# hvasbath/beat

Hardware: AMD Instinct MI355X
Metric: SMC chain-steps/s (FFI seismic gfstacking 400 patches x 64 targets x 4096 samples) (higher is better)
Workload: dtype f64; 1 GPU; BASELINE configs[2]: FFI seismic gfstacking, 400 patches x 64 targets x 4096 samples, library (64,400,3,25,4096) f64 = 62.9 GB in HBM, nearest_neighbor, covariance scalar; population SURVEY 8(d): nucleation U over the 20x20 fault, time 0; chains_per_gpu=512, global_chains=512, parallelism=chains sharded over 1 GPU(s), library replicated

## Files before the change

beat_amd/_lib.py:

```python
import ctypes as C
import os

import numpy as np

_HERE = os.path.dirname(os.path.abspath(__file__))
LIB_PATH = os.environ.get("BEATAMD_LIB") or os.path.join(_HERE, "libbeat_amd.so")

NEAREST_NEIGHBOR, MULTILINEAR = 0, 1
W_SCALAR, W_DENSE = 0, 1
STF_HALF_SINUSOID = 0
POL_MTQT, POL_MT, POL_DC = 0, 1, 2
INTERPOLATIONS = {"nearest_neighbor": NEAREST_NEIGHBOR, "multilinear": MULTILINEAR}

OK, EINVAL, EHIP, EINDEX, ENOMEM, ENAN, ENOTPSD, EBADCOV, EOUTSIDE = 0, -1, -2, -3, -4, -5, -6, -7, -8
ABI_VERSION = 120


class BeatAmdError(RuntimeError):
    pass


class FfiLayout(C.Structure):
    _fields_ = [
        ("nparams", C.c_int64),
# ... 6 lines not shown
        ("time_off", C.c_int64),
        ("h_laplacian_off", C.c_int64),
    ]


_vp, _i32, _i64, _f64 = C.c_void_p, C.c_int32, C.c_int64, C.c_double
_pi32, _pi64 = C.POINTER(C.c_int32), C.POINTER(C.c_int64)

_PROTOS = {
    "beatamd_ctx_create": [C.c_int, C.POINTER(_vp)],
    "beatamd_ctx_destroy": [_vp],
    "beatamd_ctx_set_stream": [_vp, _vp],
    "beatamd_ctx_use_own_stream": [_vp],
    "beatamd_ctx_synchronize": [_vp],
    "beatamd_ctx_set_step_counter": [_vp, _vp],
    "beatamd_ctx_enable_timing": [_vp, C.c_int],
    "beatamd_ctx_kernel_time": [_vp, C.c_char_p, C.POINTER(_f64), _pi64],
    "beatamd_ctx_reset_timing": [_vp],
    "beatamd_fast_sweep_batch": [_vp, _vp, _f64, _vp, _vp, _i32, _i32, _i64, _vp],
    "beatamd_seis_gflib_create": [_vp, _i64, _i64, _i64, _i64, _i64, _f64, _f64, _f64, _f64, _pi32],
    "beatamd_seis_gflib_upload": [_vp, _i32, _vp, _i64, _i64],
    "beatamd_seis_gflib_adopt": [_vp, _i32, _vp],
    "beatamd_seis_gflib_round_to_f32": [_vp, _i32],
    "beatamd_ffi_model_set_f32": [_vp, _i32, _i32, _i32],
    "beatamd_seis_gflib_device_ptr": [_vp, _i32, C.POINTER(_vp)],
    "beatamd_seis_gflib_destroy": [_vp, _i32],
    "beatamd_seis_stack_all_batch": [_vp, _i32, _i64, _vp, _vp, _vp, _i32, _vp],
    "beatamd_geo_gflib_create": [_vp, _i64, _i64, _vp, _pi32],
    "beatamd_geo_gflib_destroy": [_vp, _i32],
    "beatamd_geo_stack_all_batch": [_vp, _i32, _i64, _vp, _i32, _vp],
    "beatamd_geo_ensemble_create": [_vp, _vp, _i64, _i64, _pi32],
    "beatamd_geo_ensemble_destroy": [_vp, _i32],
    "beatamd_geo_ensemble_stack": [_vp, _i32, _vp, _vp],
    "beatamd_pred_covariance_batch": [_vp, _i64, _i64, _vp, _i64, _vp, _vp, _vp],
    "beatamd_weights_create": [_vp, _i32, _i64, _i64, _vp, _vp, _pi32],
    "beatamd_weights_update": [_vp, _i32, _i32, _i64, _vp, _vp],
    "beatamd_weights_destroy": [_vp, _i32],
    "beatamd_weights_band": [_vp, _i32, _pi64],
    "beatamd_weights_band_info": [_vp, _i32, _pi64, C.POINTER(_f64)],
    "beatamd_mvn_chol_logp_batch": [_vp, _i32, _i64, _vp, _vp, _vp],
    "beatamd_laplacian_create": [_vp, _i64, _vp, _f64, _pi32],
    "beatamd_laplacian_destroy": [_vp, _i32],
    "beatamd_laplacian_logp_batch": [_vp, _i32, _i64, _i64, _vp, _vp, _vp],
    "beatamd_ffi_model_create": [_vp, C.POINTER(FfiLayout), _i32, _vp, _vp, _vp, _pi32],
    "beatamd_ffi_model_add_wavemap": [_vp, _i32, _vp, _vp, _i32, _vp, _vp, _i32],
    "beatamd_ffi_model_add_wavemap_spectrum": [_vp, _i32, _vp, _vp, _i32, _vp, _vp, _i32, _i64, _i64, _i64],
    "beatamd_amp_spectrum_batch": [_vp, _i64, _i64, _i64, _i64, _i64, _vp, _vp, _i64, _vp],
    "beatamd_ffi_model_add_geodetic": [_vp, _i32, _vp, _vp, _vp, _i32, _vp, _vp, _vp],
    "beatamd_ffi_model_add_geodetic_geometry": [_vp, _i32, _i32, _vp, _vp, _vp, _i64, _vp, _vp, _vp, _f64,
                                                _vp, _vp, _i32, _vp, _vp, _vp],
    "beatamd_ffi_model_add_geodetic_corrections": [_vp, _i32, _i32, _vp, _vp, _vp, _vp, _vp],
    "beatamd_ffi_model_add_geodetic_corrections_kinds": [_vp, _i32, _i32, _vp, _vp, _vp, _vp, _vp, _vp, _vp],
    "beatamd_pole_coefficients_batch": [_vp, _i64, _i64, _vp, _i32, _vp, _vp, _vp, _vp],
    "beatamd_pole_coupling_batch": [_vp, _i64, _i64, _vp, _vp, _vp, _vp, _i64, _vp, _i64, _vp, _vp],
    "beatamd_ffi_model_add_polarity": [_vp, _i32, _i32, _vp, _vp, _i32, _vp, _vp, _vp, _f64, _vp, _vp, _i64, _vp, _vp],
    "beatamd_mt6_batch": [_vp, _i32, _i64, _i64, _vp, _vp, _vp, _i64, _vp, _vp, _vp],
    "beatamd_polarity_amplitudes_batch": [_vp, _i32, _i64, _i64, _vp, _vp, _vp, _i64, _vp, _vp, _i64, _vp, _vp],
    "beatamd_w_to_beta_batch": [_vp, _i64, _vp, _i64, _vp, _vp, _vp],
    "beatamd_ffi_model_set_laplacian": [_vp, _i32, _i32],
    "beatamd_ffi_model_nllk": [_vp, _i32, _pi64],
    "beatamd_ffi_model_destroy": [_vp, _i32],
    "beatamd_ffi_logp_batch": [_vp, _i32, _i64, _vp, _vp],
    "beatamd_ffi_start_times_batch": [_vp, _i32, _i64, _vp, _vp, _vp],
    "beatamd_ffi_magnitudes_batch": [_vp, _i32, _i64, _vp, _vp, _vp, _i32, _vp, _vp],
    "beatamd_ffi_moment_rate_spans_batch": [_vp, _i32, _i64, _vp, _vp, _vp, _f64, _vp],
    "beatamd_ffi_moment_rates_batch": [_vp, _i32, _i64, _vp, _vp, _vp, _i32, _vp, _vp, _f64, _i32, _i64, _i64, _vp, _vp],
    "beatamd_ffi_synthetics_batch": [_vp, _i32, _i32, _i64, _vp, _i32, _vp],
    "beatamd_ffi_astep_batch": [_vp, _i32, _i64, _vp, _vp, _vp, _vp, _vp, _vp, _vp, _f64, _vp],
    "beatamd_autocovariance_batch": [_vp, _i64, _i64, _vp, _vp, _vp],
    "beatamd_scaled_toeplitz_batch": [_vp, _i64, _i64, _vp, _vp, _vp],
    "beatamd_ball_rms_batch": [_vp, _i64, _vp, _vp, _vp, _f64, _vp, _vp, _vp],
    "beatamd_ffi_astep_batch_betas": [_vp, _i32, _i64, _vp, _vp, _vp, _vp, _vp, _vp, _vp, _vp, _vp],
    "beatamd_ffi_mstep_batch": [_vp, _i32, _i64, _vp, _vp, _vp, _i64, _i32, _i32, C.c_uint64, C.c_uint32, _i64,
                                _vp, _vp, _vp, _f64, _vp, _vp, _vp, _vp],
    "beatamd_ctx_last_kernel": [_vp, C.c_char_p, _i64],
    "beatamd_ctx_gf_group_stats": [_vp, _pi64, C.POINTER(_f64), _pi64, _pi64],
    "beatamd_ctx_gf_plan": [_vp, C.c_char_p, _i64, C.POINTER(_f64), _pi64],
    "beatamd_ctx_gf_tune_log": [_vp, C.c_char_p, _i64],
    "beatamd_gf_patch_ranges": [_i64, _i64, _i64, C.c_int32],
    "beatamd_fast_sweep_lds": [_i32, _pi32],
    "beatamd_seis_gflib_set_split_targets": [_vp, _i32, _i64],
    "beatamd_ctx_reload_knobs": [_vp],
    "beatamd_ctx_gf_chain_groups": [_vp, _i64, _vp, _vp, _i64, _vp],
    "beatamd_smc_calc_beta": [_vp, _i64, _vp, _i64, _f64, _f64, C.POINTER(_f64), _vp],
    "beatamd_smc_stage_weights": [_vp, _i64, _vp, _i64, _f64, _vp],
    "beatamd_smc_resample": [_vp, _i64, _vp, _f64, _vp],
    "beatamd_smc_population_factor": [_vp, _i64, _i64, _vp, _vp, _vp],
    "beatamd_proposal_draw": [_vp, _i64, _i64, _i64, _vp, C.c_uint64, C.c_uint32, _i64, _i32, _vp, _vp],
    "beatamd_proposal_draw_univariate": [_vp, _i64, _i64, _i32, _vp, C.c_uint64, C.c_uint32, _i64, _vp, _vp],
    "beatamd_proposal_draw_grouped": [_vp, _i64, _i64, _i64, _i64, _vp, C.c_uint64, C.c_uint32, _i64, _i32, _vp, _vp],
    "beatamd_ffi_mstep_batch_grouped": [_vp, _i32, _i64, _i64, _vp, _vp, _vp, _i64, _i32, C.c_uint64, C.c_uint32, _i64,
                                        _vp, _vp, _vp, _f64, _vp, _vp, _vp, _vp],
    "beatamd_group_moments_reset": [_vp, _i64, _i64, _vp, _i64, _vp, _vp],
    "beatamd_group_moments_update": [_vp, _i64, _i64, _i64, _vp, _vp, _i64, _vp, _vp],
    "beatamd_group_moments_factor": [_vp, _i64, _i64, _vp, _vp, _vp, _vp],
    "beatamd_gather_rows": [_vp, _i64, _i64, _vp, _i64, _vp, _vp],
    "beatamd_metropolis_tune": [_vp, _i64, _vp, _vp, _i32],
    "beatamd_ffi_model_nterm": [_vp, _i32, _pi64],
    "beatamd_ffi_llks_batch": [_vp, _i32, _i64, _vp, _vp],
    "beatamd_hyper_model_create": [_vp, _i64, _i64, _vp, _vp, _vp, _vp, _i32, _vp, _pi32],
    "beatamd_hyper_model_destroy": [_vp, _i32],
    "beatamd_hyper_logp_batch": [_vp, _i32, _i64, _vp, _vp, _vp],
    "beatamd_hyper_chain_batch": [_vp, _i32, _i64, _i64, _vp, _vp, _vp, _vp, _vp, _vp, _vp, _i32, _vp, C.c_uint64,
                                  C.c_uint32, _i64, _i32, _i32, _i32, _vp, _vp],
    "beatamd_wset_quad_batch": [_vp, _i32, _i64, _vp, _vp],
    "beatamd_ffi_obs_quads": [_vp, _i32, _vp],
    "beatamd_ffi_variance_reductions_batch": [_vp, _i32, _i64, _vp, _vp],
    "beatamd_ffi_geo_residuals_batch": [_vp, _i32, _i64, _vp, _i32, _vp],
    "beatamd_standardize_batch": [_vp, _i32, _vp, _i64, _i64, _i64, _vp, _vp, _vp],
    "beatamd_ensemble_moments_update": [_vp, _i64, _i64, _vp, _vp, _i64],
    "beatamd_ensemble_moments_finish": [_vp, _i64, _vp, _i64, _vp, _vp, _vp, _vp],
    "beatamd_trace_density_update": [_vp, _i64, _i64, _i64, _vp, _vp, _f64, _vp, _i64, _i64, _f64, _vp],
    "beatamd_trace_density_update_ranges": [_vp, _i64, _i64, _i64, _vp, _vp, _f64, _vp, _vp, _i64, _i64, _f64, _vp],
    "beatamd_like_assemble": [_vp, _i64, _i64, _i64, _vp, _vp, _vp, _i64, _i64, _i64, _i64, _i32, _vp, _vp],
    "beatamd_metropolis_propose": [_vp, _i64, _i64, _vp, _vp, _vp, _vp, _vp, _vp, _vp],
    "beatamd_metropolis_accept": [_vp, _i64, _i64, _i64, _vp, _vp, _vp, _vp, _vp, _vp, _f64, _vp, _vp],
    "beatamd_whiten_rows": [_vp, _vp, _i64, _i64, _vp],
    "beatamd_whiten_rows_batch": [_vp, _vp, _i64, _i64, _i64, _vp],
    "beatamd_chol_inverse_batch": [_vp, _i64, _i64, _vp, _vp, _vp],
    "beatamd_chol_inverse_batch_flags": [_vp, _i64, _i64, _vp, _vp, _vp, _vp],
    "beatamd_whitening_ratio_batch": [_vp, _i64, _i64, _vp, _vp, _vp],
    "beatamd_unwhiten_traces": [_vp, _i64, _i64, _vp, _vp],
    "beatamd_factor_compact": [_vp, _i64, _i64, _vp, _vp],
    "beatamd_ffi_model_update_data": [_vp, _i32, _i32, _vp],
    "beatamd_halfspace_displacements_batch": [_vp, _i64, _i32, _vp, _vp, _i64, _vp, _vp, _f64, _vp],
    "beatamd_ffi_model_set_lsq_variables": [_vp, _i32, _i32, _i32],
    "beatamd_ffi_lsq_normal_batch": [_vp, _i32, _i64, _vp, _vp, _vp, _vp],
    "beatamd_nnls_batch": [_vp, _i64, _i64, _vp, _vp, _vp, _vp, _vp],
    "beatamd_ffi_lsq_solution_batch": [_vp, _i32, _i64, _vp, _vp, _vp, _vp],
    "beatamd_geo_gf_library": [_vp, _i64, _vp, _i64, _vp, _vp, _vp, _vp, _f64, _vp],
    "beatamd_smoothing_correlated": [_vp, _i64, _vp, _i32, _vp],
    "beatamd_model_resolution": [_vp, _i64, _i64, _vp, _vp, _f64, _vp, _vp],
    "beatamd_division_rating": [_vp, _i64, _i64, _vp, _vp, _vp, _vp, _f64, _vp, _vp, _vp, _vp],
    "beatamd_column_sort": [_vp, _i64, _i64, _vp, _i64, _vp, _vp, _pi64],
    "beatamd_column_percentiles": [_vp, _i64, _i64, _vp, _i64, _vp, _vp],
    "beatamd_column_histograms": [_vp, _i64, _i64, _vp, _i64, _vp, _vp],
    "beatamd_pair_hist2d": [_vp, _i64, _i64, _vp, _i64, _vp, _i32, _i32, _vp, _vp, _vp, _pi64],
    "beatamd_pair_kde2d": [_vp, _i64, _i64, _vp, _i64, _vp, _i32, _i32, _i32, _i32, _vp, _vp, _vp, _pi64],
    "beatamd_unit_vector_sum": [_vp, _i64, _vp, _vp, _i32, _vp],
    "beatamd_spherical_kde": [_vp, _i64, _vp, _vp, _i64, _vp, _vp, _f64, _f64, _i32, _vp],
    "beatamd_mt_decompose": [_vp, _i64, _i32, _vp, _vp, _vp, _vp, _vp, _vp, _vp, _vp],
    "beatamd_fuzzy_amps": [_vp, _i64, _i32, _vp, _i64, _vp, _vp, _i32, _i32, _i32, _i32, _vp],
    "beatamd_stf_table": [_vp, _i64, _vp, _f64, _i64, _vp, _vp],
    "beatamd_trace_filter_batch": [_vp, _i64, _i64, _vp, _i64, _i64, _vp, _vp, _i32, _vp, _vp, _vp, _vp],
    "beatamd_seis_library_fill": [_vp, _i64, _i64, _i64, _vp, _i64, _i64, _vp, _vp, _i32, _vp, _vp, _vp, _i64, _i64, _vp, _vp,
                                  _i64, _vp],
    "beatamd_rupture_minmax": [_vp, _i64, _i64, _vp, _i32, _vp, _vp],
    "beatamd_contour_count": [_vp, _i64, _i64, _vp, _i32, _vp, _vp, _vp, _vp],
    "beatamd_contour_fill": [_vp, _i64, _i64, _vp, _i32, _vp, _i64, _vp, _i64, _vp, _vp, _vp, _vp, _vp, _i64, _i64, _vp, _vp],
    "beatamd_polyline_density": [_vp, _i64, _vp, _i64, _vp, _i64, _vp, _vp, _i64, _i64, _f64, _vp, _vp],
    "beatamd_autocov_lags_batch": [_vp, _i64, _i64, _vp, _i64, _i64, _vp],
    "beatamd_rank_normalize": [_vp, _i64, _vp, _vp, _vp],
    "beatamd_convergence_summary": [_vp, _i64, _i64, _i64, _vp, _i64, _vp, _f64, _f64, _i64, _i64, _vp, _vp, _pi64],
}

EXPORTS = sorted(list(_PROTOS) + ["beatamd_last_error", "beatamd_version"])

_lib = None


def load():
    global _lib
    if _lib is None:
        if not os.path.exists(LIB_PATH):
            raise BeatAmdError(
                "%s not found: build it with `python -c 'import __graft_entry__ as g; g.build()'` "
# ... 52 lines not shown
```

beat_amd/csrc/capi.cpp:

```cpp
#include <cstdlib>

#include "model.hpp"

using namespace beatamd;

namespace {

template <class T>
int32_t add_obj(std::vector<std::unique_ptr<T>> &v, std::unique_ptr<T> o)
{
    for (size_t i = 0; i < v.size(); i++)
        if (!v[i]) {
            v[i] = std::move(o);
            return (int32_t)i;
        }
    v.push_back(std::move(o));
    return (int32_t)v.size() - 1;
}

template <class T>
int host_copy(beatamd_ctx *ctx, const T *p, size_t n, std::vector<T> &out)
{
    out.resize(n);
    if (n == 0) return BEATAMD_OK;
// ... 2047 lines not shown
    BA_TRY(ctx->scratch(SL_PARTIAL, (size_t)total, &d_pmax));
    BA_TRY(ctx->scratch(SL_MISC, (size_t)nd, &d_sets));
    BA_HIP(hipMemcpyAsync(d_sets, sets.data(), sets.size() * sizeof(BallSet), hipMemcpyHostToDevice, ctx->stream));
    BA_TRY(launch_ball_rms(ctx, nd, nmax, d_sets, d_c, d_d, max_dist_perc, d_pmax, d_r, d_n, d_s));
    BA_HIP(hipStreamSynchronize(ctx->stream));
    return st.finish();
}

int beatamd_ctx_last_kernel(beatamd_ctx *ctx, char *buf, int64_t buflen)
{
    BA_CHECK(ctx && buf && buflen > 0, BEATAMD_EINVAL, "last_kernel: bad argument");
    snprintf(buf, (size_t)buflen, "%s", ctx->last_gf_kernel);
    return BEATAMD_OK;
}

int beatamd_ctx_gf_group_stats(beatamd_ctx *ctx, int64_t *chains_per_group, double *mean_rows,
                               int64_t *max_rows, int64_t *row_bytes)
{
    ENTER(ctx);
    BA_CHECK(chains_per_group && mean_rows && max_rows && row_bytes, BEATAMD_EINVAL,
             "gf_group_stats: NULL argument");
    *chains_per_group = ctx->gs_cg;
    *mean_rows = 0.0;
    *max_rows = 0;
    *row_bytes = 0;
    if (ctx->gs_ngtp == 0) return BEATAMD_OK;
    int64_t tot = 0;
    BA_TRY(gs_counters(ctx, 0, &tot, max_rows));
    *mean_rows = (double)tot / (double)ctx->gs_ngtp;
    *row_bytes = (int64_t)((double)tot * ctx->gs_trep) * ctx->gs_N * 8 * ctx->gs_nvar;
    return BEATAMD_OK;
}

int beatamd_ctx_gf_plan(beatamd_ctx *ctx, char *buf, int64_t buflen, double *mean_passes, int64_t *max_passes)
{
    ENTER(ctx);
    BA_CHECK(buf && buflen > 0, BEATAMD_EINVAL, "gf_plan: bad argument");
    snprintf(buf, (size_t)buflen, "%s", ctx->gf_plan);
    if (mean_passes) *mean_passes = ctx->gs_ngtp ? 1.0 : 0.0;
    if (max_passes) *max_passes = ctx->gs_ngtp ? 1 : 0;
    if (!ctx->gs_has_passes || ctx->gs_ngtp == 0 || (!mean_passes && !max_passes)) return BEATAMD_OK;
    int64_t tot = 0, mx = 0;
    BA_TRY(gs_counters(ctx, 1, &tot, &mx));
    if (mean_passes) *mean_passes = (double)tot / (double)ctx->gs_ngtp;
    if (max_passes) *max_passes = mx;
    return BEATAMD_OK;
}

int beatamd_ctx_gf_tune_log(beatamd_ctx *ctx, char *buf, int64_t buflen)
{
    ENTER(ctx);
    BA_CHECK(buf && buflen > 0, BEATAMD_EINVAL, "gf_tune_log: bad argument");
    snprintf(buf, (size_t)buflen, "%s", ctx->gf_tune_log);
    return BEATAMD_OK;
}

int32_t beatamd_gf_patch_ranges(int64_t ntargets, int64_t npatches, int64_t nsamples, int32_t num_cu)
{
    if (ntargets <= 0 || npatches <= 0 || nsamples <= 0) return 1;
    return (int32_t)gf_patch_ranges(ntargets, npatches, nsamples, num_cu > 0 ? num_cu : 256);
}

int32_t beatamd_fast_sweep_lds(int32_t ncells, int32_t *waves)
{
    if (ncells <= 0 || ncells > SWEEP_MAX_CELLS) return -1;
    const SweepLdsPlan pl = sweep_lds_plan(ncells);
    if (waves) *waves = pl.waves;
    return (int32_t)pl.bytes;
}

int beatamd_ctx_gf_chain_groups(beatamd_ctx *ctx, int64_t C, const double *key0, const double *key1,
                                int64_t chains_per_group, uint32_t *members)
{
    ENTER(ctx);
    BA_CHECK(C > 0 && key0 && key1 && members && chains_per_group > 0, BEATAMD_EINVAL, "gf_chain_groups: bad argument");
    const int64_t ngroups = (C + chains_per_group - 1) / chains_per_group;
    const ChainVec key[2] = {ChainVec{key0, 1, 0}, ChainVec{key1, 1, 0}};
    const uint32_t *m = nullptr;
    BA_TRY(launch_chain_members(ctx, C, key, chains_per_group, ngroups, &m));
    BA_CHECK(m != nullptr, BEATAMD_EINVAL, "gf_chain_groups: groups of more than 8192 chains are not cut");
    BA_HIP(hipStreamSynchronize(ctx->stream));
    BA_HIP(hipMemcpy(members, m, (size_t)(ngroups * chains_per_group) * sizeof(uint32_t), hipMemcpyDeviceToHost));
    return BEATAMD_OK;
}

int beatamd_smc_calc_beta(beatamd_ctx *ctx, int64_t C, const double *likelihoods, int64_t stride,
                          double beta, double coef_variation, double *beta_new, double *weights)
{
    ENTER(ctx);
    BA_CHECK(likelihoods && beta_new && weights && C > 0 && stride > 0, BEATAMD_EINVAL,
             "smc_calc_beta: bad argument");
    BA_CHECK(2.0 - beta > 1e-6, BEATAMD_EINVAL, "smc_calc_beta: beta = %g leaves no tempering step below 2", beta);
    Staging st(ctx);
    const double *d_l;
    double *d_w, *d_out;
    BA_TRY(st.in(likelihoods, (size_t)((C - 1) * stride + 1), &d_l));
    BA_TRY(st.out(weights, (size_t)C, &d_w));
    BA_TRY(ctx->scratch(SL_STAGE2, 8, &d_out));
    BA_TRY(launch_smc_calc_beta(ctx, C, d_l, stride, beta, coef_variation, 0, 0.0, d_out, d_w));
    double out[2];
    BA_HIP(hipMemcpyAsync(out, d_out, sizeof(out), hipMemcpyDeviceToHost, ctx->stream));
    BA_TRY(st.finish());
    BA_HIP(hipStreamSynchronize(ctx->stream));
    *beta_new = out[0];
    return BEATAMD_OK;
}

int beatamd_smc_stage_weights(beatamd_ctx *ctx, int64_t C, const double *likelihoods, int64_t stride,
                              double dbeta, double *weights)
{
    ENTER(ctx);
    BA_CHECK(likelihoods && weights && C > 0 && stride > 0, BEATAMD_EINVAL, "smc_stage_weights: bad argument");
    Staging st(ctx);
    const double *d_l;
    double *d_w, *d_out;
    BA_TRY(st.in(likelihoods, (size_t)((C - 1) * stride + 1), &d_l));
    BA_TRY(st.out(weights, (size_t)C, &d_w));
    BA_TRY(ctx->scratch(SL_STAGE2, 8, &d_out));
    BA_TRY(launch_smc_calc_beta(ctx, C, d_l, stride, 0.0, 0.0, 1, dbeta, d_out, d_w));
    return st.finish();
}

int beatamd_smc_resample(beatamd_ctx *ctx, int64_t C, const double *weights, double aux,
                         int32_t *indexes)
{
    ENTER(ctx);
    BA_CHECK(weights && indexes && C > 0, BEATAMD_EINVAL, "smc_resample: bad argument");
    BA_CHECK(C < (int64_t)0x7fffffff, BEATAMD_EINVAL, "smc_resample: too many chains");
    Staging st(ctx);
    const double *d_w;
    int32_t *d_i;
    double *cum;
    BA_TRY(st.in(weights, (size_t)C, &d_w));
    BA_TRY(st.out(indexes, (size_t)C, &d_i));
    BA_TRY(ctx->scratch(SL_CUM, (size_t)C, &cum));
    BA_TRY(launch_smc_resample(ctx, C, d_w, aux, cum, d_i));
    return st.finish();
}

int beatamd_smc_population_factor(beatamd_ctx *ctx, int64_t C, int64_t nparams,
                                  const double *population, const double *weights, double *factor)
{
    ENTER(ctx);
    BA_CHECK(population && weights && factor && C > 0 && nparams > 0, BEATAMD_EINVAL,
             "smc_population_factor: bad argument");
    Staging st(ctx);
    const double *d_x, *d_w;
    double *d_f;
    BA_TRY(st.in(population, (size_t)C * nparams, &d_x));
    BA_TRY(st.in(weights, (size_t)C, &d_w));
    BA_TRY(st.out(factor, (size_t)C * nparams, &d_f));
    BA_TRY(launch_pop_factor(ctx, C, nparams, d_x, nparams, d_w, d_f));
    return st.finish();
}

int beatamd_proposal_draw(beatamd_ctx *ctx, int64_t C, int64_t K, int64_t nparams,
                          const double *factor, uint64_t seed, uint32_t step, int64_t first_chain,
                          int32_t df, double *delta, double *log_u)
{
    ENTER(ctx);
    BA_CHECK(factor && delta && C >= 0 && K > 0 && nparams > 0 && df >= 0 && first_chain >= 0,
             BEATAMD_EINVAL, "proposal_draw: bad argument");
    BA_CHECK(df <= 64, BEATAMD_EINVAL, "proposal_draw: at most 64 degrees of freedom");
    if (C == 0) return BEATAMD_OK;
    Staging st(ctx);
    const double *d_f;
// ... 1022 lines not shown
```

beat_amd/csrc/ctx.hpp:

```cpp
#pragma once
#include <hip/hip_runtime.h>

#include <cstdarg>
#include <cstdint>
#include <cstdio>
#include <cstring>
#include <map>
#include <memory>
#include <string>
#include <vector>

#include "../../include/beat_amd.h"

struct beatamd_ctx;

namespace beatamd {

void set_error(const char *fmt, ...);

#define BA_HIP(expr)                                                                         \
    do {                                                                                     \
        hipError_t e_ = (expr);                                                              \
        if (e_ != hipSuccess) {                                                              \
            beatamd::set_error("%s:%d: %s -> %s", __FILE__, __LINE__, #expr,                 \
// ... 209 lines not shown
    DevMem<double> utab, btab;
};

struct FfiModel {
    beatamd_ffi_layout layout;
    int32_t nsub = 0;
    std::vector<int32_t> ndip, nstrike, patch_off;
    std::vector<double> patch_size;
    int64_t P = 0;
    DevMem<int32_t> d_ndip, d_nstrike, d_patch_off;
    DevMem<double> d_patch_size;
    std::vector<Wavemap> wavemaps;
    bool has_geo = false;
    Geodetic geo;
    bool geo_is_geometry = false;
    GeomSources geom;
    bool has_pol = false;
    Polarity pol;
    int32_t lap = -1;
    int64_t nllk() const;
    bool obs_quads_valid = false;
    std::vector<double> obs_quads;
    DevMem<double> d_obs_quads;
    int32_t lsq_var = -1, lsq_zero_var = -1;
    bool lsq_blocks_valid = false;
    DevMem<double> lsq_GG, lsq_LtL;
};

struct HyperModel {
    int64_t nterm = 0, nh = 0;
    DevMem<double> M, slog;
    DevMem<int32_t> kind, hp_index;
    int32_t ngroups = 0, group_end[8] = {0, 0, 0, 0, 0, 0, 0, 0};
};

constexpr int KNOB_UNSET = -2147483647;
#define BEATAMD_GF_KNOBS(X) \
    X(gf_kernel, "BEATAMD_GF_KERNEL") X(gs_cg, "BEATAMD_GS_CG") X(gs_ws, "BEATAMD_GS_WS") X(gs_dma, "BEATAMD_GS_DMA") X(gs_nt, "BEATAMD_GS_NT") \
    X(ws_map, "BEATAMD_WS_MAP") X(gs_pair, "BEATAMD_GS_PAIR") X(gs_nthint, "BEATAMD_GS_NTHINT") X(gs_order, "BEATAMD_GS_ORDER") \
    X(gs_fit, "BEATAMD_GS_FIT") X(gs_win, "BEATAMD_GS_WIN") X(gf_tinv, "BEATAMD_GF_TINV") X(gs_tune, "BEATAMD_GS_TUNE") \
    X(gf_order, "BEATAMD_GF_ORDER") X(gf_cgroup, "BEATAMD_GF_CGROUP") X(gs_ml, "BEATAMD_GS_ML") X(gc_global, "BEATAMD_GC_GLOBAL") \
    X(gc_sort, "BEATAMD_GC_SORT") X(gc_keys, "BEATAMD_GC_KEYS") X(gc_bands, "BEATAMD_GC_BANDS") X(gr_cap, "BEATAMD_GR_CAP") \
    X(gr_pass_alloc, "BEATAMD_GR_PASS_ALLOC") X(gr_var, "BEATAMD_GR_VAR") X(sweep_v1, "BEATAMD_SWEEP_V1") X(qf_band, "BEATAMD_QF_BAND") \
    X(qf_fuse, "BEATAMD_QF_FUSE") X(gf_split, "BEATAMD_GF_SPLIT") X(gm_wave, "BEATAMD_GM_WAVE") X(skip_parked, "BEATAMD_SKIP_PARKED") \
    X(td_strip, "BEATAMD_TD_STRIP") X(pd_strip, "BEATAMD_PD_STRIP") X(pd_rows, "BEATAMD_PD_ROWS")
struct GfKnobs {
#define X(member, env) int member = KNOB_UNSET;
    BEATAMD_GF_KNOBS(X)
#undef X
    void read_env();
    static int get(int v, int dflt) { return v == KNOB_UNSET ? dflt : v; }
    static bool is(int v, int x) { return v != KNOB_UNSET && v == x; }
    static bool set(int v) { return v != KNOB_UNSET; }
};

struct KTimer {
    double total_ms = 0;
    int64_t n = 0;
    std::vector<std::pair<hipEvent_t, hipEvent_t>> pending;
};

}

struct beatamd_ctx {
    int device = 0;
    hipStream_t stream = nullptr, own_stream = nullptr;
    bool timing = false;
    std::map<std::string, beatamd::KTimer> timers;
    std::vector<hipEvent_t> event_pool;
    int *d_status = nullptr;
    std::vector<beatamd::DevBuf> scratch_bufs;
    std::vector<std::unique_ptr<beatamd::SeisStore>> seislibs;
    std::vector<std::unique_ptr<beatamd::GeoLib>> geolibs;
    std::vector<std::unique_ptr<beatamd::GeoEnsemble>> geoens;
    std::vector<std::unique_ptr<beatamd::WeightSet>> wsets;
    std::vector<std::unique_ptr<beatamd::Laplacian>> laps;
    std::vector<std::unique_ptr<beatamd::FfiModel>> models;
    std::vector<std::unique_ptr<beatamd::HyperModel>> hypers;
    int num_cu = 256;
    char last_gf_kernel[96] = "";
    int64_t gs_ngtp = 0, gs_N = 0;
    double gs_trep = 1;
    int gs_nvar = 1;
    bool gs_has_passes = false;
    char gf_plan[384] = "";
    char gf_tune_log[512] = "";
    uint32_t *h_umax = nullptr;
    hipEvent_t umax_event = nullptr;
    bool umax_pending = false;
    int umax_hist = -1, umax_hist_cg = 0;
    std::map<std::vector<int64_t>, std::pair<int, int>> gs_tuned;
    int gs_cg = 0;
    beatamd::GfKnobs knobs;
    bool knobs_live = false;
    uint32_t *step_dev = nullptr;
    std::map<int64_t, beatamd::DevMem<double>> twiddles;

    int get_scratch(int slot, size_t bytes, void **out);
    template <class T>
    int scratch(int slot, size_t n, T **out)
    {
        void *raw = nullptr;
        const int rc = get_scratch(slot, n * sizeof(T), &raw);
        *out = static_cast<T *>(raw);
        return rc;
    }
    hipEvent_t get_event();
    void time_begin(const char *name);
    void time_end(const char *name);
    int check_status();
};

namespace beatamd {

bool is_device_ptr(const void *p);
const GfKnobs &gf_knobs(beatamd_ctx *ctx);

enum Slot : int {
    SL_IN0 = 0, SL_IN1, SL_IN2, SL_IN3, SL_IN4, SL_IN5, SL_IN6, SL_IN7,
    SL_OUT0, SL_OUT1, SL_OUT2, SL_OUT3, SL_OUT4, SL_OUT5, SL_OUT6, SL_OUT7,
    SL_ROWOFF, SL_WEIGHTS, SL_ST0, SL_RESID, SL_PARTIAL, SL_PARTIAL2, SL_QUAD, SL_MU, SL_SLIPS,
    SL_QPROP, SL_LPROP, SL_MISC, SL_GS_UROWS, SL_GS_UCOUNT, SL_GS_SLOT, SL_GS_W, SL_GS_UMAX, SL_GS_USLOT,
    SL_CHAINBAD, SL_Z, SL_ROWSCALE, SL_CUM, SL_STAGE2, SL_WHITEN,
    SL_CHOL_A, SL_CHOL_X, SL_CHOL_D, SL_CHOL_T, SL_CHOL_L,
    SL_GC_ORDER, SL_GS_ORDER, SL_GC_STREAM, SL_GC_HDR, SL_GC_META, SL_DELTA, SL_LOGU, SL_EDGES, SL_TSLOT, SL_SPLIT, SL_WS_PACK,
    SL_GM_W, SL_GM_SCALE, SL_GM_FLAG, SL_LSQ_N, SL_LSQ_B, SL_LSQ_X, SL_LSQ_U, SL_MR_SPANS,
    SL_RES_GG, SL_RES_N, SL_RES_W, SL_RES_T, SL_RES_U, SL_RATE_DMIN, SL_SPEC,
    SL_MG_FLAG, SL_MG_MOM, SL_MG_PAR, SL_MG_GRID, SL_MG_W, SL_MG_BOX,
    SL_MC_FLAG, SL_MC_COUNT, SL_MC_SUM, SL_PD_BOX,
    SL_CV_W, SL_CV_SA, SL_CV_SB, SL_CV_Q, SL_CV_CM, SL_CV_RM, SL_CV_OFF, SL_CV_ESS, SL_CV_ACT, SL_CV_STATE, SL_CV_MAC0, SL_CV_MAC1,
    SL_CV_AC, SL_CV_RHO, SL_CV_PART, SL_COUNT
};
constexpr int SL_NIN = SL_OUT0 - SL_IN0, SL_NOUT = SL_ROWOFF - SL_OUT0;

class Staging {
    beatamd_ctx *ctx;
    int nin = 0, nout = 0, nback = 0;
    struct { void *host, *dev; size_t bytes; } back[SL_NOUT];
    int in_bytes(const void *p, size_t bytes, const void **dev);
    int out_bytes(void *p, size_t bytes, void **dev, bool preload);

public:
    explicit Staging(beatamd_ctx *c) : ctx(c) {}
    template <class T>
    int in(const T *p, size_t n, const T **dev)
    {
        const void *d = nullptr;
        BA_TRY(in_bytes(p, n * sizeof(T), &d));
        *dev = static_cast<const T *>(d);
        return BEATAMD_OK;
    }
    template <class T>
    int out(T *p, size_t n, T **dev, bool preload = false)
    {
        void *d = nullptr;
        BA_TRY(out_bytes(p, n * sizeof(T), &d, preload));
        *dev = static_cast<T *>(d);
        return BEATAMD_OK;
    }
    int finish();
};

struct ScopedTimer {
    beatamd_ctx *c;
    const char *n;
    ScopedTimer(beatamd_ctx *ctx, const char *name) : c(ctx), n(name) { c->time_begin(n); }
// ... 5 lines not shown
```

beat_amd/csrc/gfshared.hip:

```cpp
#include "kernels.hpp"
#include "misfit.hpp"
#include "wave.hpp"

namespace beatamd {

constexpr int GS_NT_MAX = 64;
constexpr int GS_NTHINT_DEFAULT = 1;
constexpr int GS_WS_DEFAULT = 1;

struct GroupTabArgs {
    int nrow, nvar, CG;
    int64_t C, T, P, DS;
    const uint32_t *rowoff;
    const double *fac;
    ChainVec slips[4];
    int ucap, ustride;
    uint32_t *urows;
    uint32_t *uent;
    int nissue;
    int windowed;
    int depth;
    uint32_t *ucount;
    uint32_t *umax;
    uint16_t *slot;
// ... 676 lines not shown
k_gfstack_dmaf(GsArgs a)
{
    constexpr int GS_NT = 64;
    constexpr int GS_PITCH = GS_NT + 2;
    constexpr int KPRE = WAVES >= 4 ? 64 / WAVES : 8;
    extern __shared__ __attribute__((aligned(16))) double xbuf[];
    constexpr int CG = WAVES * 64;
    const int tid = threadIdx.x, lane = tid & 63;
    const int wave = __builtin_amdgcn_readfirstlane(tid >> 6);
    if (a.guard_mode && ((a.guard_mode == 1) == (*a.guard_umax > (uint32_t)a.guard_fit))) return;
    GS_BLOCK_DECODE(a, g, t, tile)
    int64_t gt, tbase;
    gs_table_cell(a, g, t, gt, tbase);
    const int64_t c = g * CG + tid;
    const int64_t N = a.N;
    const int64_t n0 = (int64_t)tile * GS_NT;
    GS_DMA_SETUP(1, 4, float, G32)
    for (int s = 0; s < nsteps; s++) {
        GS_DMA_STEP_TOP()
#pragma unroll
        for (int k = 0; k < NROW; k++) {
            const uint32_t xs = lds0 + (uint32_t)((gbuf + (int)sl[k] * GS_PITCH) * 4);
            const double w = wl[k];
            constexpr int NG = GS_NT / 8;
            v2f ya[4], yb[4];
            lds_rd4_pair<1, 0>(ya, xs, s);
            lds_rd4_pair<1, 32>(yb, xs, s);
            __builtin_amdgcn_sched_barrier(0);
#pragma unroll
            for (int gq = 0; gq < NG; gq++) {
                v2f(&cur)[4] = (gq & 1) ? yb : ya;
                if (gq + 1 < NG) lds_wait4_pair<4>(cur); else lds_wait4_pair<0>(cur);
                __builtin_amdgcn_sched_barrier(0);
#pragma unroll
                for (int q = 0; q < 4; q++) {
                    acc[gq * 8 + 2 * q] = fma((double)cur[q].x, w, acc[gq * 8 + 2 * q]);
                    acc[gq * 8 + 2 * q + 1] = fma((double)cur[q].y, w, acc[gq * 8 + 2 * q + 1]);
                }
                __builtin_amdgcn_sched_barrier(0);
                if (gq + 2 < NG) switch (gq + 2) {
                case 2: lds_rd4_pair<1, 64>(cur, xs, s); break;
                case 3: lds_rd4_pair<1, 96>(cur, xs, s); break;
                case 4: lds_rd4_pair<1, 128>(cur, xs, s); break;
                case 5: lds_rd4_pair<1, 160>(cur, xs, s); break;
                case 6: lds_rd4_pair<1, 192>(cur, xs, s); break;
                case 7: lds_rd4_pair<1, 224>(cur, xs, s); break;
                default: break;
                }
                __builtin_amdgcn_sched_barrier(0);
            }
        }
    }
    GS_DMA_FINISH()
}



#define BA_FMA8 \
    "v_fmac_f64 %0, %8, %16\n\tv_fmac_f64 %1, %9, %16\n\tv_fmac_f64 %2, %10, %16\n\tv_fmac_f64 %3, %11, %16\n\t" \
    "v_fmac_f64 %4, %12, %16\n\tv_fmac_f64 %5, %13, %16\n\tv_fmac_f64 %6, %14, %16\n\tv_fmac_f64 %7, %15, %16\n\t"
#define BA_RD8(OFF) \
    "ds_read_b64 %8, %17 offset:" #OFF "\n\tds_read_b64 %9, %17 offset:" #OFF "+8\n\t" \
    "ds_read_b64 %10, %17 offset:" #OFF "+16\n\tds_read_b64 %11, %17 offset:" #OFF "+24\n\t" \
    "ds_read_b64 %12, %17 offset:" #OFF "+32\n\tds_read_b64 %13, %17 offset:" #OFF "+40\n\t" \
    "ds_read_b64 %14, %17 offset:" #OFF "+48\n\tds_read_b64 %15, %17 offset:" #OFF "+56"
#define BA_ACC8(G) \
    "+v"(acc[G * 8]), "+v"(acc[G * 8 + 1]), "+v"(acc[G * 8 + 2]), "+v"(acc[G * 8 + 3]), "+v"(acc[G * 8 + 4]), \
        "+v"(acc[G * 8 + 5]), "+v"(acc[G * 8 + 6]), "+v"(acc[G * 8 + 7])
#define BA_Y8(Y) "+v"(Y[0]), "+v"(Y[1]), "+v"(Y[2]), "+v"(Y[3]), "+v"(Y[4]), "+v"(Y[5]), "+v"(Y[6]), "+v"(Y[7])
#define BA_FMA4A \
    "v_fmac_f64 %0, %8, %16\n\tv_fmac_f64 %1, %9, %16\n\tv_fmac_f64 %2, %10, %16\n\tv_fmac_f64 %3, %11, %16\n\t"
#define BA_FMA4B \
    "v_fmac_f64 %4, %12, %16\n\tv_fmac_f64 %5, %13, %16\n\tv_fmac_f64 %6, %14, %16\n\tv_fmac_f64 %7, %15, %16\n\t"
#define BA_RD4A(OFF) \
    "ds_read_b64 %8, %17 offset:" #OFF "\n\tds_read_b64 %9, %17 offset:" #OFF "+8\n\t" \
    "ds_read_b64 %10, %17 offset:" #OFF "+16\n\tds_read_b64 %11, %17 offset:" #OFF "+24\n\t"
#define BA_RD4B(OFF) \
    "ds_read_b64 %12, %17 offset:" #OFF "+32\n\tds_read_b64 %13, %17 offset:" #OFF "+40\n\t" \
    "ds_read_b64 %14, %17 offset:" #OFF "+48\n\tds_read_b64 %15, %17 offset:" #OFF "+56"
#define BA_GROUP(G, Y, OFFNEXT) \
    asm("s_waitcnt lgkmcnt(12)\n\t" BA_FMA4A BA_RD4A(OFFNEXT) "s_waitcnt lgkmcnt(12)\n\t" BA_FMA4B BA_RD4B(OFFNEXT) \
        : BA_ACC8(G), BA_Y8(Y) : "v"(w), "v"(xs))

template <int NROW, int MODE, int NB, int NTH>
__global__ void __launch_bounds__(768) __attribute__((amdgpu_waves_per_eu(3, 3)))
k_gfstack_ws(GsArgs a)
{
    constexpr int CW = 8, LW = 4;
    constexpr int GS_NT = 64;
    constexpr int GS_PITCH = GS_NT + 1;
    constexpr int KPRE = 16;
    extern __shared__ __attribute__((aligned(16))) double xbuf[];
    constexpr int CG = CW * 64;
    const int tid = threadIdx.x, lane = tid & 63;
    const int wave = __builtin_amdgcn_readfirstlane(tid >> 6);
    GS_BLOCK_DECODE(a, g, t, tile)
    int64_t gt, tbase;
    gs_table_cell(a, g, t, gt, tbase);
    const int64_t N = a.N;
    const int64_t n0 = (int64_t)tile * GS_NT;
    const uint32_t lds0 = (uint32_t)(uintptr_t)(__attribute__((address_space(3))) void *)xbuf;
    const int bufsz = (a.ucap + 1) * GS_PITCH;
    const int P = a.nv ? (int)__builtin_amdgcn_readfirstlane((int)a.nv[gt]) : (int)a.P;
    const int nvar = a.nvar;
    const int nsteps = P * nvar;

    if (wave >= CW) {
        GS_LOADER_PROGRAM(0, 8, double, G_a = a.G[iv] + tbase)
        return;
    }

    static_assert(NROW == 1, "the loader / consumer kernel exists for single-row interpolation");
    const int64_t c = a.order ? (int64_t)a.order[g * CG + tid] : g * CG + tid;
    for (int i = tid; i < NB * GS_PITCH; i += CG) xbuf[(i / GS_PITCH) * bufsz + a.ucap * GS_PITCH + (i % GS_PITCH)] = 0.0;
    __builtin_amdgcn_fence(__ATOMIC_RELEASE, "workgroup");
    double acc[GS_NT];
#pragma unroll
    for (int i = 0; i < GS_NT; i++) acc[i] = 0.0;
    uint32_t sl_n;
    double wl_n;
    const uint32_t voff_s = (uint32_t)tid * 2u;
    const char *const slot_base = reinterpret_cast<const char *>(a.slot + (gt * a.vmax) * CG);
    const char *const w_base = reinterpret_cast<const char *>(a.w + (gt * a.vmax) * CG);
    const uint32_t slot_step = (uint32_t)(CG * 2);
    const uint32_t w_step = (uint32_t)(CG * 8);
    const int64_t w_var_bytes = a.w_var_stride * 8;
    auto tab_slot = [&](int p) { return slot_base + (uint32_t)p * slot_step; };
    auto tab_w = [&](int p, int iv) {
        return w_base + (uint32_t)p * w_step + (nvar == 1 ? (int64_t)0 : (int64_t)iv * w_var_bytes);
    };
    auto fetch_tabs = [&](const char *ps, const char *pw) {
        asm("global_load_ushort %0, %1, %2" : "=v"(sl_n) : "v"(voff_s), "s"(ps));
        uint32_t voff_w;
        asm("v_lshlrev_b32 %1, 2, %2\n\t"
            "global_load_dwordx2 %0, %1, %3" : "=v"(wl_n), "=&v"(voff_w) : "v"(voff_s), "s"(pw));
    };
    auto row_address = [&](uint32_t base) {
        uint32_t x;
        asm("s_waitcnt vmcnt(0)\n\t"
            "v_lshl_add_u32 %0, %1, 6, %1\n\t"
            "v_lshl_add_u32 %0, %0, 3, %2" : "=&v"(x) : "v"(sl_n), "s"(base), "v"(wl_n));
        return x;
    };
    auto landed_weight = [&](uint32_t after) {
        double x;
        asm("v_mov_b64 %0, %1" : "=v"(x) : "v"(wl_n), "v"(after));
        return x;
    };
    static_assert(GS_PITCH == 65, "row_address multiplies by 65");
    constexpr int NG8 = GS_NT / 8;
    static_assert(NG8 == 8, "the read schedule below is written for 64-sample tiles");
    double ya[8], yb[8];
    int p1 = 0, iv1 = 0;
    gs_advance(p1, iv1, P, nvar);
    int gbuf = 0;
    const int ring = NB * bufsz;
    double w;
    uint32_t xs;
    if (__ballot(c < a.C) == 0) {
        for (int s = 0; s <= nsteps; s++) __builtin_amdgcn_s_barrier();
    } else {
    fetch_tabs(tab_slot(0), tab_w(0, 0));
    xs = row_address(lds0);
    w = landed_weight(xs);
    __builtin_amdgcn_sched_barrier(0);
    __builtin_amdgcn_s_barrier();
    __builtin_amdgcn_sched_barrier(0);
    lds_rd8_b64<0>(ya, xs, -1);
    lds_rd8_b64<64>(yb, xs, -1);
    __builtin_amdgcn_sched_barrier(0);
    fetch_tabs(tab_slot(p1), tab_w(p1, iv1));
    gs_advance(p1, iv1, P, nvar);
    const char *ps_run = tab_slot(p1), *pw_run = tab_w(p1, iv1);
    int iv_run = iv1;
    const int64_t dw_next = (nvar == 1) ? (int64_t)w_step : w_var_bytes;
    const int64_t dw_wrap = (int64_t)w_step - (int64_t)(nvar - 1) * w_var_bytes;
#pragma clang loop unroll(disable)
    for (int s = 0; s < nsteps; s++) {
        int gnext = gbuf + bufsz;
        if (gnext == ring) gnext = 0;
        __builtin_amdgcn_sched_barrier(0);
        BA_GROUP(0, ya, 128);
        BA_GROUP(1, yb, 192);
        BA_GROUP(2, ya, 256);
        BA_GROUP(3, yb, 320);
        BA_GROUP(4, ya, 384);
        BA_GROUP(5, yb, 448);
        __builtin_amdgcn_sched_barrier(0);
        asm("s_waitcnt lgkmcnt(0)\n\t" BA_FMA8
            : BA_ACC8(6), BA_Y8(ya) : "v"(w), "v"(xs), "v"(yb[0]), "v"(yb[1]), "v"(yb[2]), "v"(yb[3]),
              "v"(yb[4]), "v"(yb[5]), "v"(yb[6]), "v"(yb[7]));
        __builtin_amdgcn_sched_barrier(0);
        gbuf = gnext;
        const uint32_t xs_n = row_address(lds0 + (uint32_t)(gbuf * 8));
        __builtin_amdgcn_sched_barrier(0);
        __builtin_amdgcn_s_barrier();
        __builtin_amdgcn_sched_barrier(0);
        lds_rd8_b64<0>(ya, xs_n, s);
        __builtin_amdgcn_sched_barrier(0);
        asm(BA_FMA8
            "v_mov_b64 %16, %18\n\t" BA_RD8(64)
            : BA_ACC8(7), BA_Y8(yb), "+v"(w) : "v"(xs_n), "v"(wl_n));
        xs = xs_n;
        __builtin_amdgcn_sched_barrier(0);
        fetch_tabs(ps_run, pw_run);
        {
            uint32_t ds;
            int64_t dw;
            asm("s_add_i32 %0, %0, 1\n\t"
                "s_cmp_eq_u32 %0, %3\n\t"
                "s_cselect_b32 %0, 0, %0\n\t"
                "s_cselect_b32 %1, %4, 0\n\t"
                "s_cselect_b64 %2, %5, %6"
                : "+s"(iv_run), "=&s"(ds), "=&s"(dw) : "s"(nvar), "s"(slot_step), "s"(dw_wrap), "s"(dw_next) : "scc");
            ps_run += ds;
            pw_run += dw;
        }
    }
    asm volatile("s_waitcnt vmcnt(0) lgkmcnt(0)"
                 : "+v"(ya[0]), "+v"(ya[1]), "+v"(ya[2]), "+v"(ya[3]), "+v"(ya[4]), "+v"(ya[5]), "+v"(ya[6]),
                   "+v"(ya[7]), "+v"(yb[0]), "+v"(yb[1]), "+v"(yb[2]), "+v"(yb[3]), "+v"(yb[4]), "+v"(yb[5]),
                   "+v"(yb[6]), "+v"(yb[7]), "+v"(sl_n), "+v"(wl_n));
    __builtin_amdgcn_sched_barrier(0);
    }

    const bool live = (c < a.C);
    const int nvalid = (int)min((int64_t)GS_NT, N - n0);
    if (MODE == GF_STORE_SYN) {
        if (live) {
            gs_store_syn<GS_NT>(a.out + (c * a.T + t) * N + n0, acc, nvalid);
        }
        return;
    }
    __builtin_amdgcn_s_barrier();
    if (tid < GS_NT) xbuf[tid] = (tid < nvalid) ? a.data[t * N + n0 + tid] : 0.0;
    if (MODE == GF_RESID_BAND1 && tid >= GS_NT && tid < 3 * GS_NT)
        xbuf[tid] = ((tid - GS_NT) >> 1) < nvalid ? a.band_w[(t * N + n0) * 2 + (tid - GS_NT)] : 0.0;
    __builtin_amdgcn_fence(__ATOMIC_RELEASE, "workgroup");
    __builtin_amdgcn_s_barrier();
    __builtin_amdgcn_fence(__ATOMIC_ACQUIRE, "workgroup");
    if (MODE == GF_RESID_BAND1) {
        const double *wbt = xbuf + GS_NT;
        const auto resid = [&](int i) { return xbuf[i] - acc[i]; };
        const double rfirst = resid(0);
        const Band1Tile tl = band1_tile<true, GS_NT>(resid, [&](int i, int b) { return wbt[2 * i + b]; }, nvalid, n0 + nvalid == N);
        if (live) {
            const int64_t e = (c * a.T + t) * a.ntile + tile;
            a.partial[e] = tl.q;
            a.edges[2 * e] = rfirst;
            a.edges[2 * e + 1] = tl.r_last;
        }
    } else if (MODE == GF_RESID_STORE) {
        constexpr int TP = 17;
        double *tw = xbuf + GS_NT + wave * (64 * TP);
        const uint32_t cu = (uint32_t)min(c, (int64_t)0xffffffff);
        const int sl = lane & 15;
#pragma unroll
        for (int i0 = 0; i0 < GS_NT; i0 += 16) {
#pragma unroll
            for (int i = 0; i < 16; i++) tw[lane * TP + i] = xbuf[i0 + i] - acc[i0 + i];
            __builtin_amdgcn_fence(__ATOMIC_RELEASE, "wavefront");
            __builtin_amdgcn_wave_barrier();
            __builtin_amdgcn_fence(__ATOMIC_ACQUIRE, "wavefront");
#pragma unroll
            for (int k = 0; k < 16; k++) {
                const double v = tw[(k * 4 + (lane >> 4)) * TP + sl];
                const int64_t cc = (int64_t)(uint32_t)__shfl((int)cu, k * 4 + (lane >> 4));
                if (cc < a.C && i0 + sl < nvalid) a.out[(cc * a.T + t) * N + n0 + i0 + sl] = v;
            }
            __builtin_amdgcn_fence(__ATOMIC_RELEASE, "wavefront");
            __builtin_amdgcn_wave_barrier();
        }
    } else {
        const double q = gs_misfit_scalar<GS_NT>(a.wscalar[t], acc, xbuf, nvalid);
        if (live) a.partial[(c * a.T + t) * a.ntile + tile] = q;
    }
}


#undef BA_GROUP
#undef BA_RD4B
#undef BA_RD4A
#undef BA_FMA4B
#undef BA_FMA4A
#undef BA_Y8
#undef BA_ACC8
#undef BA_RD8
#undef BA_FMA8

template <int F32, int MODE, int NB, int NTH>
__global__ void __launch_bounds__(768) __attribute__((amdgpu_waves_per_eu(3, 3)))
k_gfstack_wsp(GsArgs a)
{
    constexpr int CW = 8, LW = 4;
    constexpr int GS_NT = 64;
    constexpr int GS_PITCH = GS_NT + 2;
    constexpr int ES = F32 ? 4 : 8;
    typedef typename std::conditional<F32 != 0, float, double>::type elem_t;
    typedef typename std::conditional<F32 != 0, v2f, v2d>::type pair_t;
    constexpr int KPRE = 16;
    extern __shared__ __attribute__((aligned(16))) double xbuf[];
    constexpr int CG = CW * 64;
    const int tid = threadIdx.x, lane = tid & 63;
    const int wave = __builtin_amdgcn_readfirstlane(tid >> 6);
    GS_BLOCK_DECODE(a, g, t, tile)
    int64_t gt, tbase;
    gs_table_cell(a, g, t, gt, tbase);
    const int64_t N = a.N;
    const int64_t n0 = (int64_t)tile * GS_NT;
    const uint32_t lds0 = (uint32_t)(uintptr_t)(__attribute__((address_space(3))) void *)xbuf;
    const int bufsz = (a.ucap + 1) * GS_PITCH;
    const int P = a.nv ? (int)__builtin_amdgcn_readfirstlane((int)a.nv[gt]) : (int)a.P;
    const int nvar = a.nvar;
    const int nsteps = P * nvar;

    if (wave >= CW) {
        GS_LOADER_PROGRAM(F32, ES, elem_t, if constexpr (F32 != 0) G_a = a.G32[iv] + tbase; else G_a = a.G[iv] + tbase)
        return;
    }

    const int64_t c = a.order ? (int64_t)a.order[g * CG + tid] : g * CG + tid;
    for (int i = tid; i < NB * GS_PITCH; i += CG)
        reinterpret_cast<elem_t *>(xbuf)[(i / GS_PITCH) * bufsz + a.ucap * GS_PITCH + (i % GS_PITCH)] = (elem_t)0;
    __builtin_amdgcn_fence(__ATOMIC_RELEASE, "workgroup");
    double acc[GS_NT];
#pragma unroll
    for (int i = 0; i < GS_NT; i++) acc[i] = 0.0;
    uint32_t sl_n;
    double wl_n;
    const uint32_t voff_s = (uint32_t)tid * 2u;
    const char *const slot_base = reinterpret_cast<const char *>(a.slot + (gt * a.vmax) * CG);
    const char *const w_base = reinterpret_cast<const char *>(a.w + (gt * a.vmax) * CG);
    const uint32_t slot_step = (uint32_t)(CG * 2);
    const uint32_t w_step = (uint32_t)(CG * 8);
    const int64_t w_var_bytes = a.w_var_stride * 8;
    auto tab_slot = [&](int p) { return slot_base + (uint32_t)p * slot_step; };
    auto tab_w = [&](int p, int iv) {
        return w_base + (uint32_t)p * w_step + (nvar == 1 ? (int64_t)0 : (int64_t)iv * w_var_bytes);
    };
    auto fetch_tabs = [&](const char *ps, const char *pw) {
        asm("global_load_ushort %0, %1, %2" : "=v"(sl_n) : "v"(voff_s), "s"(ps));
        uint32_t voff_w;
        asm("v_lshlrev_b32 %1, 2, %2\n\t"
            "global_load_dwordx2 %0, %1, %3" : "=v"(wl_n), "=&v"(voff_w) : "v"(voff_s), "s"(pw));
    };
    auto row_address = [&](uint32_t base) {
        uint32_t x;
        asm("s_waitcnt vmcnt(0)\n\t"
            "v_lshl_add_u32 %0, %1, 5, %1\n\t"
            "v_lshl_add_u32 %0, %0, %c4, %2" : "=&v"(x) : "v"(sl_n), "s"(base), "v"(wl_n), "n"(F32 ? 3 : 4));
        return x;
    };
    auto landed_weight = [&](uint32_t after) {
        double x;
        asm("v_mov_b64 %0, %1" : "=v"(x) : "v"(wl_n), "v"(after));
        return x;
    };
    static_assert(GS_PITCH == 66, "row_address multiplies by 33 qwords");
    static_assert(GS_NT == 64, "the read schedule below is written for 64-sample tiles");
    pair_t ya[4], yb[4];
    int p1 = 0, iv1 = 0;
    gs_advance(p1, iv1, P, nvar);
    int gbuf = 0;
    const int ring = NB * bufsz;
    double w;
    uint32_t xs;
    fetch_tabs(tab_slot(0), tab_w(0, 0));
    xs = row_address(lds0);
    w = landed_weight(xs);
    __builtin_amdgcn_sched_barrier(0);
    __builtin_amdgcn_s_barrier();
    __builtin_amdgcn_sched_barrier(0);
    lds_rd4_pair<F32 ? 1 : 2, 0>(ya, xs, -1);
    lds_rd4_pair<F32 ? 1 : 2, 32>(yb, xs, -1);
    __builtin_amdgcn_sched_barrier(0);
    fetch_tabs(tab_slot(p1), tab_w(p1, iv1));
    gs_advance(p1, iv1, P, nvar);
#define F2_FMA(G, Y)                                                          \
    _Pragma("unroll") for (int q = 0; q < 4; q++) {                           \
        acc[(G) * 8 + 2 * q] = fma((double)Y[q].x, w, acc[(G) * 8 + 2 * q]);   \
        acc[(G) * 8 + 2 * q + 1] = fma((double)Y[q].y, w, acc[(G) * 8 + 2 * q + 1]); \
    }
#define F2_GROUP(G, Y, OFFNEXT)              \
    lds_wait4_pair<4>(Y);                      \
    __builtin_amdgcn_sched_barrier(0);       \
    F2_FMA(G, Y)                             \
    __builtin_amdgcn_sched_barrier(0);       \
    lds_rd4_pair<F32 ? 1 : 2, OFFNEXT>(Y, xs, s);           \
    __builtin_amdgcn_sched_barrier(0);
#pragma clang loop unroll(disable)
    for (int s = 0; s < nsteps; s++) {
        int gnext = gbuf + bufsz;
        if (gnext == ring) gnext = 0;
        const char *const ps2 = tab_slot(p1), *const pw2 = tab_w(p1, iv1);
        gs_advance(p1, iv1, P, nvar);
        __builtin_amdgcn_sched_barrier(0);
        F2_GROUP(0, ya, 64)
        F2_GROUP(1, yb, 96)
        F2_GROUP(2, ya, 128)
        F2_GROUP(3, yb, 160)
        F2_GROUP(4, ya, 192)
        F2_GROUP(5, yb, 224)
        lds_wait4_pair<0>(ya);
        lds_wait4_pair<0>(yb);
        __builtin_amdgcn_sched_barrier(0);
        F2_FMA(6, ya)
        __builtin_amdgcn_sched_barrier(0);
        gbuf = gnext;
        const uint32_t xs_n = row_address(lds0 + (uint32_t)(gbuf * ES));
        __builtin_amdgcn_sched_barrier(0);
        __builtin_amdgcn_s_barrier();
        __builtin_amdgcn_sched_barrier(0);
        lds_rd4_pair<F32 ? 1 : 2, 0>(ya, xs_n, s);
        __builtin_amdgcn_sched_barrier(0);
        F2_FMA(7, yb)
        __builtin_amdgcn_sched_barrier(0);
        w = landed_weight(xs_n);
        lds_rd4_pair<F32 ? 1 : 2, 32>(yb, xs_n, s);
        xs = xs_n;
        __builtin_amdgcn_sched_barrier(0);
        fetch_tabs(ps2, pw2);
    }
#undef F2_GROUP
#undef F2_FMA
    asm volatile("s_waitcnt vmcnt(0) lgkmcnt(0)"
                 : "+v"(ya[0]), "+v"(ya[1]), "+v"(ya[2]), "+v"(ya[3]), "+v"(yb[0]), "+v"(yb[1]), "+v"(yb[2]),
                   "+v"(yb[3]), "+v"(sl_n), "+v"(wl_n));
    __builtin_amdgcn_sched_barrier(0);

    const bool live = (c < a.C);
    const int nvalid = (int)min((int64_t)GS_NT, N - n0);
    if (MODE == GF_STORE_SYN) {
        if (live) {
            gs_store_syn<GS_NT>(a.out + (c * a.T + t) * N + n0, acc, nvalid);
        }
        return;
    }
    __builtin_amdgcn_s_barrier();
    if (tid < GS_NT) xbuf[tid] = (tid < nvalid) ? a.data[t * N + n0 + tid] : 0.0;
    __builtin_amdgcn_fence(__ATOMIC_RELEASE, "workgroup");
    __builtin_amdgcn_s_barrier();
    __builtin_amdgcn_fence(__ATOMIC_ACQUIRE, "workgroup");
    if (MODE == GF_RESID_STORE) {
        gs_resid_store<GS_NT>(a.out + (c * a.T + t) * N + n0, acc, xbuf, live, nvalid);
    } else {
        const double q = gs_misfit_scalar<GS_NT>(a.wscalar[t], acc, xbuf, nvalid);
        if (live) a.partial[(c * a.T + t) * a.ntile + tile] = q;
    }
}


template <int WAVES, int NROW, int MODE>
static int launch_shared_one(dim3 grid, size_t lds, hipStream_t s, const GsArgs &a)
{
    void (*kern)(GsArgs) = nullptr;
    if constexpr (WAVES == 16) {
        kern = k_gfstack_dma<WAVES, NROW, MODE, 32, 1>;
    } else if (a.f32pair) {
        kern = k_gfstack_dmaf<WAVES, NROW, MODE>;
    } else {
        kern = (a.dma == 2 && a.nt == 32) ? k_gfstack_dma<WAVES, NROW, MODE, 32, 1>
             : (a.dma == 2) ? k_gfstack_dma<WAVES, NROW, MODE, 64, 1>
                            : k_gfstack_dma<WAVES, NROW, MODE, 64, 0>;
    }
    if (lds > 64 * 1024)
        BA_HIP(hipFuncSetAttribute((const void *)kern, hipFuncAttributeMaxDynamicSharedMemorySize, (int)lds));
    hipLaunchKernelGGL(kern, grid, dim3(WAVES * 64), lds, s, a);
    return BEATAMD_OK;
}

template <int WAVES, int NROW>
static int launch_shared_mode(int mode, dim3 grid, size_t lds, hipStream_t s, const GsArgs &a)
{
    if (mode == GF_STORE_SYN) return launch_shared_one<WAVES, NROW, GF_STORE_SYN>(grid, lds, s, a);
    if (mode == GF_RESID_SCALAR) return launch_shared_one<WAVES, NROW, GF_RESID_SCALAR>(grid, lds, s, a);
    return launch_shared_one<WAVES, NROW, GF_RESID_STORE>(grid, lds, s, a);
}

template <int WAVES>
static int launch_shared_nrow(int nrow, int mode, dim3 grid, size_t lds, hipStream_t s,
                              const GsArgs &a)
{
    if (nrow == 1) return launch_shared_mode<WAVES, 1>(mode, grid, lds, s, a);
    return launch_shared_mode<WAVES, 4>(mode, grid, lds, s, a);
}

static int launch_ws(int mode, dim3 grid, size_t lds, hipStream_t s, const GsArgs &a, int pair)
{
    void (*kern)(GsArgs);
#define BA_WS_PICK(NAME, ...)                                                                          \
    (mode == GF_STORE_SYN ? NAME<__VA_ARGS__ GF_STORE_SYN, 3, 1>                                      \
     : mode == GF_RESID_SCALAR ? NAME<__VA_ARGS__ GF_RESID_SCALAR, 3, 1> : NAME<__VA_ARGS__ GF_RESID_STORE, 3, 1>)
#define BA_WS_PICK0(NAME, ...)                                                                         \
    (mode == GF_STORE_SYN ? NAME<__VA_ARGS__ GF_STORE_SYN, 3, 0>                                      \
     : mode == GF_RESID_SCALAR ? NAME<__VA_ARGS__ GF_RESID_SCALAR, 3, 0> : NAME<__VA_ARGS__ GF_RESID_STORE, 3, 0>)
    if (pair == 1) kern = a.nthint ? BA_WS_PICK(k_gfstack_wsp, 1,) : BA_WS_PICK0(k_gfstack_wsp, 1,);
    else if (pair == 2) kern = a.nthint ? BA_WS_PICK(k_gfstack_wsp, 0,) : BA_WS_PICK0(k_gfstack_wsp, 0,);
    else if (mode == GF_RESID_BAND1) kern = a.nthint ? k_gfstack_ws<1, GF_RESID_BAND1, 3, 1> : k_gfstack_ws<1, GF_RESID_BAND1, 3, 0>;
    else kern = a.nthint ? BA_WS_PICK(k_gfstack_ws, 1,) : BA_WS_PICK0(k_gfstack_ws, 1,);
#undef BA_WS_PICK0
#undef BA_WS_PICK
    BA_HIP(hipFuncSetAttribute((const void *)kern, hipFuncAttributeMaxDynamicSharedMemorySize, (int)lds));
    hipLaunchKernelGGL(kern, grid, dim3(768), lds, s, a);
    return BEATAMD_OK;
}

constexpr int WS_CG = 512;
constexpr int WS_LW = 4;
constexpr int WS_USTRIDE = 128;
constexpr int WS_CAP_MAX = 96;
constexpr int WS_MAXPASS = (WS_CG + WS_CAP_MAX - 1) / WS_CAP_MAX;

struct WsTabArgs {
    int nvar, cap;
    int64_t C, T, P, DS;
    int64_t vmax;
    const uint32_t *rowoff;
    ChainVec slips[4];
    const uint32_t *order;
    uint32_t *npass;
    const uint32_t *voff;
    uint32_t *utotal;
    uint32_t *ucount;
    uint32_t *uent;
    uint16_t *slot;
    double *w;
    int64_t w_var_stride;
    int64_t R;
};

__global__ void __launch_bounds__(256) k_ws_scan(const uint32_t *npass, uint32_t *voff, uint32_t *nv, int64_t P)
{
    __shared__ uint32_t part[256];
    const int tid = threadIdx.x;
    const int64_t gt = blockIdx.x;
    uint32_t run = 0;
    for (int64_t base = 0; base < P; base += 256) {
        const int64_t p = base + tid;
        const uint32_t x = p < P ? npass[gt * P + p] : 0u;
        part[tid] = x;
        __syncthreads();
        uint32_t before = 0, total = 0;
        for (int k = 0; k < 256; k++) {
            const uint32_t y = part[k];
            if (k < tid) before += y;
            total += y;
        }
        if (p < P) voff[gt * P + p] = run + before;
        run += total;
        __syncthreads();
    }
    if (tid == 0) nv[gt] = run;
}

__global__ void __launch_bounds__(WS_CG) k_ws_pack(const uint32_t *order, const int32_t *active, int64_t C, uint32_t *out)
{
    __shared__ uint32_t wsum[WS_CG / 64];
    const int tid = threadIdx.x;
    const int lane = tid & 63, wv = tid >> 6;
    const int64_t pos = (int64_t)blockIdx.x * WS_CG + tid;
    const uint32_t c = order ? order[pos] : (pos < C ? (uint32_t)pos : 0xffffffffu);
    const bool on = c != 0xffffffffu && (int64_t)c < C && active[c] != 0;
    const uint64_t m = __ballot(on);
    if (lane == 0) wsum[wv] = (uint32_t)__popcll(m);
    __syncthreads();
    uint32_t before = 0, total = 0;
    for (int q = 0; q < WS_CG / 64; q++) {
        const uint32_t x = wsum[q];
        if (q < wv) before += x;
        total += x;
    }
    uint32_t *o = out + (int64_t)blockIdx.x * WS_CG;
    if (on) o[before + (uint32_t)__popcll(m & ((1ull << lane) - 1ull))] = c;
    if ((uint32_t)tid >= total) o[tid] = 0xffffffffu;
}

constexpr int64_t WS_MAP_MAX = 16384;
template <int FILL, int MAP>
__global__ void __launch_bounds__(WS_CG) k_ws_tables(WsTabArgs a)
{
    extern __shared__ __attribute__((aligned(16))) uint16_t rowmap[];
    __shared__ __attribute__((aligned(16))) uint32_t vals[WS_CG];
    __shared__ __attribute__((aligned(16))) uint32_t firstv[WS_CG];
    __shared__ uint32_t lst[WS_CG];
    __shared__ uint32_t gm[WS_CG];
    __shared__ uint16_t slt[WS_CG];
    __shared__ uint8_t rk2i[WS_MAXPASS][128];
    __shared__ uint32_t wsum[WS_CG / 64 + 1];
    const int tid = threadIdx.x;
    const int lane = tid & 63, wv = tid >> 6;
    const int64_t gtp = xcd_items8(blockIdx.x, gridDim.x);
    const int64_t p = gtp % a.P;
    const int64_t gt = gtp / a.P;
    const int64_t t = gt % a.T;
    const int64_t g = gt / a.T;
    const int64_t pos_in_batch = g * WS_CG + tid;
    const uint32_t oc = a.order ? a.order[pos_in_batch] : (uint32_t)pos_in_batch;
    const bool live = pos_in_batch < a.C && oc != 0xffffffffu;
    const int64_t c = live ? (int64_t)oc : 0;
    const uint32_t v = live ? a.rowoff[(c * a.T + t) * a.P + p] : 0xffffffffu;
    double sl[4] = {0.0, 0.0, 0.0, 0.0};
    if constexpr (FILL)
        for (int iv = 0; iv < a.nvar; iv++)
            if (live) sl[iv] = a.slips[iv].base[c * a.slips[iv].stride + a.slips[iv].off + (t % a.R) * a.P + p];
    gm[tid] = 0;
    uint32_t pos = 0, U = 0;
    bool first = false;
    if constexpr (MAP) {
        const uint32_t row0 = (uint32_t)((t * a.P + p) * a.DS);
        for (int64_t i = tid; i < a.DS; i += WS_CG) rowmap[i] = 0;
        __syncthreads();
        if (live) rowmap[v - row0] = 1;
        __syncthreads();
        uint32_t run = 0;
        for (int64_t base = 0; base < a.DS; base += WS_CG) {
            const int64_t i = base + tid;
            const uint32_t f = (i < a.DS) ? rowmap[i] : 0u;
            const uint64_t m = __ballot(f != 0);
            if (lane == 0) wsum[wv] = (uint32_t)__popcll(m);
            __syncthreads();
            uint32_t before = 0, total = 0;
            for (int q = 0; q < WS_CG / 64; q++) {
                const uint32_t x = wsum[q];
                if (q < wv) before += x;
                total += x;
            }
            if (f) {
                const uint32_t ps = run + before + (uint32_t)__popcll(m & ((1ull << lane) - 1ull));
                rowmap[i] = (uint16_t)ps;
                if constexpr (FILL) lst[ps] = row0 + (uint32_t)i;
            }
            run += total;
            __syncthreads();
        }
        U = run;
        if (live) pos = rowmap[v - row0];
    } else {
        vals[tid] = v;
        __syncthreads();
        first = live;
        {
            const uint4 *v4 = reinterpret_cast<const uint4 *>(vals);
            for (int k4 = 0; k4 < WS_CG / 4; k4++) {
                const uint4 x = v4[k4];
                const int k = 4 * k4;
                first = first && !((x.x == v && k < tid) || (x.y == v && k + 1 < tid) || (x.z == v && k + 2 < tid) ||
                                   (x.w == v && k + 3 < tid));
            }
        }
        firstv[tid] = first ? v : 0xffffffffu;
        {
            const uint64_t m = __ballot(first);
            if (lane == 0) wsum[wv] = (uint32_t)__popcll(m);
        }
        __syncthreads();
        if (live) {
            const uint4 *f4 = reinterpret_cast<const uint4 *>(firstv);
            for (int k4 = 0; k4 < WS_CG / 4; k4++) {
                const uint4 x = f4[k4];
                pos += (x.x < v) + (x.y < v) + (x.z < v) + (x.w < v);
            }
        }
        for (int q = 0; q < WS_CG / 64; q++) U += wsum[q];
    }
    const int npass = U == 0 ? 1 : (int)((U + (uint32_t)a.cap - 1) / (uint32_t)a.cap);
    if constexpr (!FILL) {
        if (tid == 0) {
            a.npass[gtp] = (uint32_t)npass;
            a.utotal[gtp] = U;
        }
        return;
    }
    if (tid == 0) a.utotal[gtp] = U;
    const int per = U == 0 ? 1 : ((int)U + npass - 1) / npass;
    if constexpr (!MAP) {
        if (first) lst[pos] = v;
    }
    if (live) atomicOr(&gm[pos], 1u << (tid >> 5));
    __syncthreads();
    const int mypass = live ? (int)pos / per : -1;
    if (wv < npass) {
        const int base = wv * per;
        const int n = min(per, (int)U - base);
        if (n <= 32) {
            if (lane < n) slt[base + lane] = (uint16_t)lane;
        } else {
            const int depth = a.cap / 32;
            const int r0 = lane, r1 = lane + 64;
            const uint32_t m0 = r0 < n ? gm[base + r0] : 0u, m1 = r1 < n ? gm[base + r1] : 0u;
            const int key0 = r0 < n ? ((__popc(m0) << 8) | (255 - r0)) : -1;
            const int key1 = r1 < n ? ((__popc(m1) << 8) | (255 - r1)) : -1;
            int rank0 = 0, rank1 = 0;
            for (int j = 0; j < n; j++) {
                const int kj = (__popc(gm[base + j]) << 8) | (255 - j);
                rank0 += kj > key0;
                rank1 += kj > key1;
            }
            if (r0 < n && rank0 < 32) slt[base + r0] = (uint16_t)rank0;
            if (r1 < n && rank1 < 32) slt[base + r1] = (uint16_t)rank1;
            if (r0 < n) rk2i[wv][rank0] = (uint8_t)r0;
            if (r1 < n) rk2i[wv][rank1] = (uint8_t)r1;
            wave_lds_sync();
            uint32_t wmask = 0;
            int wcnt = 0;
            if (lane < 32) {
                wmask = gm[base + rk2i[wv][lane]];
                wcnt = 1;
            }
            for (int rk = 32; rk < n; rk++) {
                const int ridx = (int)rk2i[wv][rk];
                const uint32_t mm = gm[base + ridx];
                int cost = (lane < 32 && wcnt < depth) ? ((__popc(wmask & mm) << 12) | (wcnt << 6) | lane) : 0x7fffffff;
                cost = wave_butterfly<OpMin>(cost);
                const int w = cost & 63;
                if (lane == w) {
                    slt[base + ridx] = (uint16_t)(w + 32 * wcnt);
                    wmask |= mm;
                    wcnt++;
                }
            }
        }
    }
    __syncthreads();
    const int64_t v0 = gt * a.vmax + (a.voff ? (int64_t)a.voff[gtp] : p);
    const uint16_t myslot = live ? slt[pos] : (uint16_t)0;
    constexpr int kstr = WS_USTRIDE / WS_LW;
    for (int k = 0; k < npass; k++) {
        const int64_t vs = v0 + k;
        const int base = k * per;
        const int n = min(per, (int)U - base);
        const bool mine = mypass == k;
        a.slot[vs * WS_CG + tid] = mine ? myslot : (uint16_t)a.cap;
        for (int iv = 0; iv < a.nvar; iv++) a.w[(int64_t)iv * a.w_var_stride + vs * WS_CG + tid] = mine ? sl[iv] : 0.0;
        if (tid == 0) a.ucount[vs] = (uint32_t)n;
        if (tid < WS_USTRIDE) {
            const int j = tid;
            uint32_t *e = a.uent + ((vs * WS_LW + (j % WS_LW)) * kstr + (j / WS_LW)) * 2;
            e[0] = n > 0 ? lst[base + (j < n ? j : n - 1)] : 0u;
            e[1] = j < n ? (uint32_t)slt[base + j] : 0u;
        }
    }
}

static int pick_group(int64_t C)
{
    const int cand[4] = {512, 256, 128, 64};
    const double cost[4] = {2.55, 1.5, 1.2, 1.0};
    int best = 64;
    double bestc = 1e300;
    for (int i = 0; i < 4; i++) {
        const double c = (double)((C + cand[i] - 1) / cand[i]) * cost[i];
        if (c < bestc - 1e-12) { bestc = c; best = cand[i]; }
    }
    return best;
}

static bool shared_fit(const GfStackCall &k, const GfPlan &p, int cg, bool row_passes, int *ucap_out)
{
    const SeisLib &L = *k.libs[0];
    const int64_t DS = L.D * L.S;
    const int64_t ucap = std::min<int64_t>((int64_t)cg * p.nrow, DS);
    if (!row_passes) {
        if (2 * ucap * (GS_NT_MAX + 2) * 8 > 158 * 1024) return false;
        if (2 * DS * 4 + cg * 4 + 2048 > 60 * 1024) return false;
    }
    *ucap_out = (int)std::max<int64_t>(ucap, 2);
    return true;
}

GfGroup gfstack_group(const GfPlan &p, int cg, int ucap)
{
    GfGroup g;
    g.cg = cg; g.ucap = ucap;
    g.ws = p.ws512 && cg == WS_CG;
    g.mode = p.mode;
    if (p.mode == GF_RESID_BAND1) g.band1 = gf_band1(g.ws && !p.f32 && !p.pair64 && p.fused, GF_BY_WS, &g.mode);
    return g;
}

bool gfstack_shared_plan(const GfStackCall &k, GfPlan &p)
{
    const SeisLib &L = *k.libs[0];
    if (L.N % 2 != 0) return false;
    const GfKnobs &kn = *p.knobs;
    if (GfKnobs::is(kn.gf_kernel, 0)) return false;
    if (!GfKnobs::is(kn.gf_kernel, 1) && k.C < 48) return false;
    p.ws512 = GfKnobs::get(kn.gs_ws, GS_WS_DEFAULT) != 0 && k.interp != BEATAMD_MULTILINEAR && L.N % 2 == 0 &&
              !(GfKnobs::set(kn.gs_dma) && kn.gs_dma != 2) && !(GfKnobs::set(kn.gs_nt) && kn.gs_nt != 64);
    int cg = pick_group(k.C);
    const int gq = GfKnobs::get(kn.gs_cg, 0);
    if (gq == 64 || gq == 128 || gq == 256 || gq == 512 || gq == 1024) cg = gq;
    if (p.R > 1) {
        if (!p.ws512) return false;
        cg = WS_CG;
    }
    const bool ws = p.ws512 && cg == WS_CG;
    while (!ws && std::min<int64_t>((int64_t)cg * p.nrow, L.D * L.S) * (GS_NT_MAX + 2) * 8 > 72 * 1024 && cg > 64) cg /= 2;
    int ucap = 0;
    if (!shared_fit(k, p, cg, ws, &ucap)) return false;
    p.group = gfstack_group(p, cg, ucap);
    p.tune = !GfKnobs::set(kn.gs_cg) && !GfKnobs::is(kn.gs_tune, 0);
    const int cand[4] = {512, 256, 128, 64};
    for (int i = 0; i < 4 && p.tune; i++) {
        if (p.R > 1 && cand[i] != 512) continue;
        if (cand[i] > 64 && (int64_t)cand[i] / 2 >= k.C) continue;
        if (k.C >= 1024 && cand[i] < 256) continue;
        if (k.C >= 384 && cand[i] < 128) continue;
        int u = 0;
        if (shared_fit(k, p, cand[i], p.ws512 && cand[i] == WS_CG, &u)) p.cand[p.ncand++] = gfstack_group(p, cand[i], u);
    }
    return true;
}

static void gs_common_args(GsArgs &a, const GfStackCall &k, const GfPlan &p, const GfLaunch &ln, int64_t ngroups)
{
    const GfKnobs &kn = *p.knobs;
    const SeisLib &L = *k.libs[0];
    memset(&a, 0, sizeof(a));
    for (int v = 0; v < k.nvar; v++) {
        a.G[v] = k.libs[v]->g;
        a.G32[v] = k.libs[v]->g32;
    }
    a.nvar = k.nvar;
    a.C = k.C; a.T = L.T; a.P = L.P; a.N = L.N;
    a.Ttab = p.Ttab; a.rows_per_target = L.P * L.D * L.S;
    a.tslot = ln.tslot;
    a.ngroups = ngroups;
    a.data = k.data; a.wscalar = k.wscalar; a.out = k.out;
    a.nthint = GfKnobs::set(kn.gs_nthint) ? (kn.gs_nthint != 0) : (GS_NTHINT_DEFAULT && ngroups == 1);
}

static int64_t gs_grid(GsArgs &a, const GfKnobs &kn)
{
    a.xcd_order = (a.ngroups > 1 && !GfKnobs::is(kn.gs_order, 0)) ? 1 : 0;
    if (GfKnobs::is(kn.gs_order, 1)) a.xcd_order = 1;
    return a.xcd_order ? ((a.T * a.ntile + 7) / 8) * 8 * a.ngroups : a.ngroups * a.T * a.ntile;
}

void gs_record_stats(beatamd_ctx *ctx, const GfStackCall &k, int64_t GTP, int64_t Ttab, int cg, bool has_passes)
{
    ctx->gs_ngtp = GTP;
    ctx->gs_trep = (double)k.libs[0]->T / (double)Ttab;
    ctx->gs_N = k.libs[0]->N;
    ctx->gs_cg = cg;
    ctx->gs_nvar = k.nvar;
    ctx->gs_has_passes = has_passes;
}

static int launch_gfstack_ws(beatamd_ctx *ctx, const GfStackCall &k, const GfPlan &p, const GfLaunch &ln, const GfGroup &g)
{
    const GfKnobs &kn = *p.knobs;
    const SeisLib &L = *k.libs[0];
    const int64_t Ttab = p.Ttab;
    const int mode = g.mode;
    const int64_t ngroups = (k.C + WS_CG - 1) / WS_CG;
    const int64_t GT = ngroups * Ttab, GTP = GT * L.P;
    const int64_t bound = std::min<int64_t>(WS_CG, L.D * L.S);
    const int cap = bound <= 32 ? 32 : bound <= 64 ? 64 : WS_CAP_MAX;
    const int maxpass = (int)((bound + cap - 1) / cap);
    const int64_t vmax = L.P * maxpass;

    WsTabArgs ta;
    memset(&ta, 0, sizeof(ta));
    ta.nvar = k.nvar; ta.cap = cap;
    ta.C = k.C; ta.T = Ttab; ta.P = L.P; ta.DS = L.D * L.S; ta.vmax = vmax;
    ta.rowoff = ln.rowoff;
    for (int v = 0; v < k.nvar; v++) ta.slips[v] = k.slips[v];
    ta.R = p.R;
    if (ngroups > 1 && k.order_key[0].base && k.order_key[1].base && GfKnobs::get(kn.gc_global, 1) != 0)
        BA_TRY(launch_chain_members(ctx, k.C, k.order_key, WS_CG, ngroups, &ta.order, GfKnobs::get(kn.gc_global, 1) == 2));
    BA_TRY(ctx->scratch(SL_GS_UCOUNT, (size_t)(3 * GTP + GT), &ta.utotal));
    ta.npass = ta.utotal + GTP;
    uint32_t *voff = ta.npass + GTP, *nv = voff + GTP;
    const size_t nvs = (size_t)GT * vmax + 3;
    BA_TRY(ctx->scratch(SL_GS_UROWS, nvs, &ta.ucount));
    BA_TRY(ctx->scratch(SL_GS_USLOT, nvs * WS_USTRIDE * 2, &ta.uent));
    BA_TRY(ctx->scratch(SL_GS_SLOT, nvs * WS_CG, &ta.slot));
    ta.w_var_stride = (int64_t)GT * vmax * WS_CG;
    BA_TRY(ctx->scratch(SL_GS_W, (size_t)ta.w_var_stride * k.nvar + (size_t)3 * WS_CG, &ta.w));
    {
        ScopedTimer tm(ctx, "grouptables");
        if (k.active) {
            uint32_t *packed;
            BA_TRY(ctx->scratch(SL_WS_PACK, (size_t)ngroups * WS_CG, &packed));
            hipLaunchKernelGGL(k_ws_pack, dim3((unsigned)ngroups), dim3(WS_CG), 0, ctx->stream, ta.order, k.active, k.C, packed);
            ta.order = packed;
        }
        const bool map = ta.DS <= WS_MAP_MAX && !GfKnobs::is(kn.ws_map, 0);
        const size_t mlds = map ? (size_t)ta.DS * sizeof(uint16_t) : 0;
        if (maxpass > 1) {
            if (map) hipLaunchKernelGGL((k_ws_tables<0, 1>), dim3((unsigned)GTP), dim3(WS_CG), mlds, ctx->stream, ta);
            else hipLaunchKernelGGL((k_ws_tables<0, 0>), dim3((unsigned)GTP), dim3(WS_CG), 0, ctx->stream, ta);
            hipLaunchKernelGGL(k_ws_scan, dim3((unsigned)GT), dim3(256), 0, ctx->stream, ta.npass, voff, nv, L.P);
            ta.voff = voff;
        }
        if (map) hipLaunchKernelGGL((k_ws_tables<1, 1>), dim3((unsigned)GTP), dim3(WS_CG), mlds, ctx->stream, ta);
        else hipLaunchKernelGGL((k_ws_tables<1, 0>), dim3((unsigned)GTP), dim3(WS_CG), 0, ctx->stream, ta);
    }
    BA_HIP(hipGetLastError());

    GsArgs a;
    const bool f32 = p.f32, pair64 = p.pair64;
    gs_common_args(a, k, p, ln, ngroups);
    a.nrow = 1;
    a.CG = WS_CG; a.ucap = cap; a.ustride = WS_USTRIDE;
    a.nt = 64; a.dma = 2; a.ws = 3;
    a.ntile = (int)((L.N + 63) / 64);
    a.nv = maxpass > 1 ? nv : nullptr;
    a.vmax = vmax;
    a.order = ta.order;
    a.uent = ta.uent; a.ucount = ta.ucount; a.slot = ta.slot; a.w = ta.w;
    a.w_var_stride = ta.w_var_stride;
    if (mode == GF_RESID_SCALAR || mode == GF_RESID_BAND1) BA_TRY(ctx->scratch(SL_PARTIAL, (size_t)k.C * L.T * a.ntile, &a.partial));
    if (mode == GF_RESID_BAND1) {
        BA_TRY(ctx->scratch(SL_EDGES, (size_t)k.C * L.T * a.ntile * 2, &a.edges));
        a.band_w = k.band_w;
    }
    const int64_t nblocks = gs_grid(a, kn);
    BA_CHECK(nblocks < (int64_t)0x7fffffff, BEATAMD_EINVAL, "gfstack: batch too large");
    size_t lds = f32 ? (size_t)(cap + 1) * (64 + 2) * sizeof(float) * 3
                     : (size_t)(cap + 1) * (64 + (pair64 ? 2 : 1)) * sizeof(double) * 3;
    lds = std::max<size_t>(lds, (64 + 8 * 64 * 17) * sizeof(double));
    BA_CHECK(lds <= 160 * 1024, BEATAMD_EINVAL, "internal: k_gfstack_ws row buffers exceed LDS");
    if (f32 || pair64)
        snprintf(ctx->last_gf_kernel, sizeof(ctx->last_gf_kernel), "k_gfstack_ws%s<%d,%d,%d>", f32 ? "32" : "p64", mode, a.ws,
                 a.nthint);
    else
        snprintf(ctx->last_gf_kernel, sizeof(ctx->last_gf_kernel), "k_gfstack_ws<%d,%d,%d,%d>", 1, mode, a.ws, a.nthint);
    snprintf(ctx->gf_plan, sizeof(ctx->gf_plan),
             "loader/consumer kernel: 512-chain groups, nearest neighbour; %d row slots per LDS buffer (a patch can touch min(512, "
             "D*S = %lld) rows), %s", cap, (long long)(L.D * L.S),
             maxpass > 1 ? "patches that touch more are staged in passes of equal size" : "one pass per patch");
    gs_record_stats(ctx, k, GTP, Ttab, WS_CG, maxpass > 1);
    {
        ScopedTimer tm(ctx, "gfstack");
        BA_TRY(launch_ws(mode, dim3((unsigned)nblocks), lds, ctx->stream, a, f32 ? 1 : (pair64 ? 2 : 0)));
    }
    BA_HIP(hipGetLastError());
    if (a.partial)
        BA_TRY(launch_sum_tiles(ctx, a.partial, k.C * L.T, a.ntile, k.quad, nullptr, 0, a.edges, k.band_w, L.T, L.N));
    return BEATAMD_OK;
}

static int launch_dma_twin(beatamd_ctx *ctx, const GfStackCall &k, const GfPlan &p, const GfGroup &g, GsArgs &shared, int twin,
                           int ucap, bool windowed, int64_t GTP)
{
    const SeisLib &L = *k.libs[0];
    const int nrow = p.nrow, CG = g.cg, mode = g.mode;
    GsArgs a = shared;
    a.ucap = ucap;
    a.guard_mode = twin;
    size_t lds = (size_t)ucap * (a.nt + 2) * sizeof(double);
    BA_CHECK(2 * lds <= 158 * 1024, BEATAMD_EINVAL, "internal: k_gfstack_dma row buffers exceed LDS");
    a.dma = GfKnobs::is(p.knobs->gs_dma, 1) ? 1 : 2;
    if (a.nt == 32 && a.dma != 2) { a.nt = 64; a.ntile = (int)((L.N + 63) / 64); lds = (size_t)ucap * (a.nt + 2) * sizeof(double); }
    BA_CHECK(CG != 1024 || a.dma == 2, BEATAMD_EINVAL, "gfstack: 1024-chain groups need the LDS-DMA kernel");
    BA_CHECK(!windowed || a.dma == 2, BEATAMD_EINVAL, "internal: window slots need the ds_read_b64 kernel");
    a.ws = 0;
    a.f32pair = 0;
    if (a.dma == 2 && a.nt == 64 && CG <= 512 && p.f32) {
        a.f32pair = 1;
        lds = std::max<size_t>((size_t)ucap * (a.nt + 2) * sizeof(float) * 2, 64 * sizeof(double));
    } else {
        lds *= 2;
    }
    const dim3 grid((unsigned)gs_grid(a, *p.knobs));
    if (a.f32pair)
        snprintf(ctx->last_gf_kernel, sizeof(ctx->last_gf_kernel), "k_gfstack_dmaf<%d,%d,%d>", CG / 64, nrow, mode);
    else
        snprintf(ctx->last_gf_kernel, sizeof(ctx->last_gf_kernel), "%s<%d,%d,%d,%d,%d>",
                 "k_gfstack_dma", CG / 64, nrow, mode, a.nt, a.dma == 2 ? 1 : 0);
    gs_record_stats(ctx, k, GTP, p.Ttab, CG, false);
    snprintf(ctx->gf_plan, sizeof(ctx->gf_plan),
             "lane <-> chain kernel with %d-chain groups (%s): row buffers of %d slots%s", CG,
             k.C < 384 ? "small batch" : nrow == 4 ? "multilinear below 192 chains or an odd sample count" : "group size measured fastest",
             ucap, twin ? " sized by the previous launch's distinct-row count" : "");
    if (CG == 1024) BA_TRY(launch_shared_nrow<16>(nrow, mode, grid, lds, ctx->stream, a));
    else if (CG == 512) BA_TRY(launch_shared_nrow<8>(nrow, mode, grid, lds, ctx->stream, a));
    else if (CG == 256) BA_TRY(launch_shared_nrow<4>(nrow, mode, grid, lds, ctx->stream, a));
    else if (CG == 128) BA_TRY(launch_shared_nrow<2>(nrow, mode, grid, lds, ctx->stream, a));
    else BA_TRY(launch_shared_nrow<1>(nrow, mode, grid, lds, ctx->stream, a));
    BA_HIP(hipGetLastError());
    shared.nt = a.nt; shared.ntile = a.ntile;
    return BEATAMD_OK;
}

int launch_gfstack_shared(beatamd_ctx *ctx, const GfStackCall &k, const GfPlan &p, const GfLaunch &ln, const GfGroup &g)
{
    if (g.ws) return launch_gfstack_ws(ctx, k, p, ln, g);
    const GfKnobs &kn = *p.knobs;
    const SeisLib &L = *k.libs[0];
    const int nrow = p.nrow, CG = g.cg, mode = g.mode;
    int ucap = g.ucap;
    const int64_t Ttab = p.Ttab;
    const int64_t ngroups = (k.C + CG - 1) / CG;
    const int64_t GTP = ngroups * Ttab * L.P;

    GroupTabArgs ga;
    memset(&ga, 0, sizeof(ga));
    ga.nrow = nrow; ga.nvar = k.nvar; ga.CG = CG;
    ga.C = k.C; ga.T = Ttab; ga.P = L.P; ga.DS = L.D * L.S;
    ga.rowoff = ln.rowoff; ga.fac = ln.fac;
    for (int v = 0; v < k.nvar; v++) ga.slips[v] = k.slips[v];
    ga.ucap = ucap;
    ga.ustride = (ucap + 63) / 64 * 64;
    BA_TRY(ctx->scratch(SL_GS_UROWS, (size_t)GTP * ga.ustride, &ga.urows));
    BA_TRY(ctx->scratch(SL_GS_USLOT, (size_t)GTP * ga.ustride * 2, &ga.uent));
    BA_TRY(ctx->scratch(SL_GS_UCOUNT, (size_t)GTP, &ga.ucount));
    BA_TRY(ctx->scratch(SL_GS_SLOT, (size_t)(GTP + 3) * nrow * CG, &ga.slot));
    ga.w_var_stride = (nrow == 1) ? ngroups * L.P * CG : GTP * 4 * CG;
    BA_TRY(ctx->scratch(SL_GS_W, (size_t)ga.w_var_stride * k.nvar + (size_t)3 * 4 * CG, &ga.w));
    const bool fit_lds = CG <= 128 && !GfKnobs::is(kn.gs_fit, 0);
    if (fit_lds) {
        BA_TRY(ctx->scratch(SL_GS_UMAX, 1, &ga.umax));
        BA_HIP(hipMemsetAsync(ga.umax, 0, sizeof(uint32_t), ctx->stream));
    }
    ga.nissue = CG / 64;
    {
        const int depth = (ucap + 31) / 32;
// ... 59 lines not shown
```

beat_amd/csrc/gfstack.hip:

```cpp
#include <cstdlib>
#include <cstring>

#include "kernels.hpp"
#include "misfit.hpp"

namespace beatamd {

struct TabArgs {
    int interp;
    int64_t C, T, P, D, S;
    double st_min, st_dt, du_min, du_dt;
    ChainVec durations;
    StartTimeSrc st;
    uint32_t *rowoff;
    double *fac;
    int *status;
    int64_t R;
};

__device__ __forceinline__ int to_int16(double x) { return (int)(int16_t)(long long)x; }

__device__ __forceinline__ bool wrap_index(int &i, int n)
{
    if (i < 0) i += n;
// ... 312 lines not shown
    const int64_t ncu = std::max(1, num_cu);
    if (walks >= 2 * ncu) return 1;
    int best = 1;
    int64_t best_cost = ((walks + ncu - 1) / ncu) * (P + 5);
    for (int d = 2; d <= 32 && P / d >= 32; d++) {
        if (P % d) continue;
        const int64_t cost = ((walks * d + ncu - 1) / ncu) * (P / d + 5);
        if (cost < best_cost) { best = d; best_cost = cost; }
    }
    return best;
}

__global__ void __launch_bounds__(256) k_split_tslot(int64_t Tv, int R, const int32_t *tslot, int32_t *out)
{
    const int64_t t = (int64_t)blockIdx.x * 256 + threadIdx.x;
    if (t < Tv) out[t] = (tslot ? tslot[t / R] : 0) * R + (int32_t)(t % R);
}

template <int MODE>
__global__ void __launch_bounds__(256) k_split_combine(const double *part, int64_t C, int64_t T, int64_t N, int R,
                                                      const double *data, const double *wscalar, double *out, double *quad,
                                                      const double *band_w)
{
    __shared__ double sq[256 + 1];
    __shared__ double tsum[4];
    const int64_t ct = blockIdx.x, t = ct % T, c = ct / T;
    const int n = threadIdx.x;
    double v = 0.0;
    if (n < N) {
        const double *pp = part + ((c * T + t) * R) * N + n;
        double syn = pp[0];
        for (int r = 1; r < R; r++) syn += pp[(int64_t)r * N];
        if (MODE == GF_STORE_SYN) out[ct * N + n] = syn;
        else if (MODE == GF_RESID_SCALAR) v = scalar_t(wscalar[t], data[t * N + n], syn);
        else if (MODE == GF_RESID_BAND1) v = data[t * N + n] - syn;
        else out[ct * N + n] = data[t * N + n] - syn;
    }
    if (MODE != GF_RESID_SCALAR && MODE != GF_RESID_BAND1) return;
    sq[n] = v;
    __syncthreads();
    const int ntile = (int)((N + 63) / 64);
    const int n0 = n * 64, nv = (int)min((int64_t)64, N - (int64_t)n0);
    __shared__ double w[MODE == GF_RESID_BAND1 ? 2 * 256 : 2];
    if (MODE == GF_RESID_BAND1) {
        if (n < N) {
            w[2 * n] = band_w[(t * N + n) * 2];
            w[2 * n + 1] = band_w[(t * N + n) * 2 + 1];
        }
        __syncthreads();
    }
    if (n < ntile) {
        const auto r = [&](int i) { return sq[n0 + i]; };
        if (MODE == GF_RESID_BAND1) tsum[n] = band1_tile<false, 64>(r, [&](int i, int b) { return w[2 * (n0 + i) + b]; }, nv, n0 + nv == N).q;
        else tsum[n] = scalar_tile<false, 64>(r, nv);
    }
    __syncthreads();
    if (n == 0) {
        double s_ = 0.0;
        for (int k = 0; k < ntile; k++) {
            const int last = k * 64 + 63;
            if (MODE == GF_RESID_BAND1 && k + 1 < ntile) s_ = band1_join(s_, tsum[k], true, w[2 * last], w[2 * last + 1], sq[last], sq[last + 1]);
            else s_ = tile_join(s_, tsum[k]);
        }
        quad[ct] = s_;
    }
}

GfPlan gf_plan_call(const GfStackCall &k, const GfKnobs &kn, int num_cu)
{
    GfPlan p;
    const SeisLib &L = *k.libs[0];
    p.knobs = &kn;
    const int split = GfKnobs::get(kn.gf_split, -1);
    p.R = split == 0 || split == 1 ? 1 : split > 1 ? ((L.P % split == 0 && L.N <= 256) ? split : 1)
                                   : gf_patch_ranges(L.split_T > 0 ? L.split_T : L.T, L.P, L.N, num_cu);
    p.T = L.T * p.R; p.P = L.P / p.R;
    p.tinv = !k.st.explicit_st && !k.st.shift_off && !GfKnobs::is(kn.gf_tinv, 0);
    p.slots = !k.st.explicit_st && k.st.shift_off && k.st.nslot > 0 && !GfKnobs::is(kn.gf_tinv, 0);
    p.Ttab = p.tinv ? p.R : p.slots ? (int64_t)k.st.nslot * p.R : p.T;
    p.nrow = k.interp == BEATAMD_MULTILINEAR ? 4 : 1;
    p.f32 = k.f32;
    for (int v = 0; v < k.nvar; v++) p.f32 = p.f32 && k.libs[v]->g32 != nullptr;
    p.pair64 = GfKnobs::is(kn.gs_pair, 1);
    p.fused = !GfKnobs::is(kn.qf_fuse, 0);
    p.mode = p.R > 1 ? (int)GF_STORE_SYN : k.mode;
    p.mode_combine = k.mode;
    if (p.R > 1 && k.mode == GF_RESID_BAND1) p.band1 = gf_band1(p.fused, GF_BY_COMBINE, &p.mode_combine);
    const bool band1 = p.mode == GF_RESID_BAND1;
    p.mode_standin = band1 ? (int)GF_RESID_STORE : p.mode;
    if (!p.f32 && gfstack_ml_applicable(k, p)) {
        p.stacker = GF_RUNS;
        p.standin_band1 = band1 && p.fused;
        if (band1) p.band1 = gf_band1(p.fused, GF_BY_RUNS, &p.mode);
    } else if (gfstack_shared_plan(k, p)) {
        p.stacker = GF_GROUPS;
    } else if (band1) {
        p.band1 = gf_band1(false, GF_BY_NONE, &p.mode);
    }
    return p;
}

static int tune_group_size(beatamd_ctx *ctx, const GfStackCall &k, const GfPlan &p, const GfLaunch &ln, GfGroup *out)
{
    const SeisLib &L = *k.libs[0];
    const int64_t cbucket = k.C < 512 ? k.C : 512 * std::min<int64_t>((k.C + 511) / 512, 16);
    const std::vector<int64_t> key = {cbucket, p.nrow, k.nvar, L.T, L.P, L.D, L.S, L.N, p.Ttab, p.f32 ? 1 : 0};
    auto it = ctx->gs_tuned.find(key);
    if (it == ctx->gs_tuned.end()) {
        const int nc = p.ncand;
        int best = -1;
        float best_ms = 0.f, ms_of[4] = {0.f, 0.f, 0.f, 0.f};
        hipEvent_t e0, e1;
        BA_HIP(hipEventCreate(&e0)); BA_HIP(hipEventCreate(&e1));
        for (int i = 0; i < nc && nc > 1; i++) {
            float ms_min = 0.f;
            for (int rep = 0; rep < 2; rep++) {
                BA_HIP(hipEventRecord(e0, ctx->stream));
                BA_TRY(launch_gfstack_shared(ctx, k, p, ln, p.cand[i]));
                BA_HIP(hipEventRecord(e1, ctx->stream));
                BA_HIP(hipEventSynchronize(e1));
                BA_HIP(hipEventElapsedTime(&ms_min, e0, e1));
            }
            ms_of[i] = ms_min;
            if (best < 0 || ms_min < best_ms) { best = i; best_ms = ms_min; }
            if (ms_min > 2.f * best_ms) break;
        }
        (void)hipEventDestroy(e0); (void)hipEventDestroy(e1);
        if (nc == 1) best = 0;
        if (best >= 0) it = ctx->gs_tuned.emplace(key, std::make_pair(p.cand[best].cg, p.cand[best].ucap)).first;
        char *w = ctx->gf_tune_log; size_t left = sizeof(ctx->gf_tune_log);
        int n = snprintf(w, left, "group size for %lld chains (T %lld, P %lld, D*S %lld, N %lld, %d row(s) per chain): ",
                         (long long)k.C, (long long)L.T, (long long)L.P, (long long)(L.D * L.S), (long long)L.N, p.nrow);
        for (int i = 0; i < nc && n > 0 && (size_t)n < left; i++) {
            w += n; left -= (size_t)n;
            n = ms_of[i] > 0.f ? snprintf(w, left, "%d: %.3f ms%s", p.cand[i].cg, ms_of[i], i + 1 < nc ? ", " : "")
                               : snprintf(w, left, "%d: %s%s", p.cand[i].cg, nc == 1 ? "only candidate" : "not timed", i + 1 < nc ? ", " : "");
        }
        if (best >= 0 && n > 0 && (size_t)n < left) { w += n; left -= (size_t)n; snprintf(w, left, " -> %d", p.cand[best].cg); }
        if (getenv("BEATAMD_VERBOSE")) fprintf(stderr, "beat_amd: %s\n", ctx->gf_tune_log);
    }
    *out = it != ctx->gs_tuned.end() ? gfstack_group(p, it->second.first, it->second.second) : p.group;
    return BEATAMD_OK;
}

static int launch_gfstack_split(beatamd_ctx *ctx, const GfStackCall &call, const GfPlan &p, GfLaunch &ln)
{
    const SeisLib &L = *call.libs[0];
    const int R = p.R;
    SeisLib views[4];
    GfStackCall v = call;
    v.active = nullptr;
    for (int i = 0; i < call.nvar; i++) {
        views[i] = *call.libs[i];
        views[i].T = p.T; views[i].P = p.P;
        v.libs[i] = &views[i];
    }
    double *part;
    BA_TRY(ctx->scratch(SL_SPLIT, (size_t)call.C * L.T * R * L.N, &part));
    v.out = part;
    v.quad = nullptr; v.data = nullptr; v.wscalar = nullptr; v.band_w = nullptr;
    BA_TRY(launch_gfstack_impl(ctx, v, p, ln));
    const size_t n0 = strlen(ctx->gf_plan);
    snprintf(ctx->gf_plan + n0, sizeof(ctx->gf_plan) - n0, "; %lld-sample traces: patches stacked in %d ranges of %lld "
             "(%lld walks instead of %lld), partial synthetics summed in range order", (long long)L.N, R, (long long)(L.P / R),
             (long long)(L.T * R * ((L.N + 63) / 64)), (long long)(L.T * ((L.N + 63) / 64)));
    const dim3 grid((unsigned)(call.C * L.T));
// ... 30 lines not shown
    }
    if ((p.stacker == GF_GROUPS && p.R == 1 ? ln.group.band1 : p.band1) == GF_BY_QUADFORM)
        BA_TRY(launch_quadform_banded(ctx, call.band_w, 1, L.N, L.T, call.C, call.out, L.T * L.N, L.N, call.quad, L.T));
    return BEATAMD_OK;
}

static int launch_gfstack_impl(beatamd_ctx *ctx, const GfStackCall &k, const GfPlan &p, GfLaunch &ln)
{
    const GfKnobs &kn = *p.knobs;
    const SeisLib &L = *k.libs[0];
    if (k.C == 0) return BEATAMD_OK;
    const int64_t R = p.R, Ttab = p.Ttab;
    ln.tslot = p.slots ? k.st.tslot : nullptr;
    if (R > 1 && (p.tinv || p.slots)) {
        int32_t *vslot;
        BA_TRY(ctx->scratch(SL_TSLOT, (size_t)L.T, &vslot));
        hipLaunchKernelGGL(k_split_tslot, dim3((unsigned)((L.T + 255) / 256)), dim3(256), 0, ctx->stream, L.T, (int)R,
                           p.slots ? k.st.tslot : nullptr, vslot);
        ln.tslot = vslot;
    }
    const int64_t CTP = k.C * Ttab * L.P;

    TabArgs ta;
    ta.interp = k.interp; ta.R = R;
    ta.C = k.C; ta.T = Ttab; ta.P = L.P; ta.D = L.D; ta.S = L.S;
    ta.st_min = L.st_min; ta.st_dt = L.st_dt; ta.du_min = L.du_min; ta.du_dt = L.du_dt;
    ta.durations = k.durations; ta.st = k.st;
    if (p.slots) ta.st.shift_off = k.st.slot_shift_off;
    ta.status = ctx->d_status;
    BA_TRY(ctx->scratch(SL_ROWOFF, (size_t)CTP * p.nrow, &ta.rowoff));
    ta.fac = nullptr;
    if (p.nrow == 4) BA_TRY(ctx->scratch(SL_WEIGHTS, (size_t)CTP * 4, &ta.fac));
    {
        ScopedTimer tm(ctx, "tables");
        hipLaunchKernelGGL(k_gf_tables, dim3((unsigned)((CTP + 255) / 256)), dim3(256), 0,
                           ctx->stream, ta);
    }
    BA_HIP(hipGetLastError());
    ln.rowoff = ta.rowoff; ln.fac = ta.fac;

    const int *standin = nullptr;
    if (p.stacker == GF_RUNS) {
        BA_TRY(launch_gfstack_ml(ctx, k, p, ln, &standin));
        if (!standin) return BEATAMD_OK;
    } else if (p.stacker == GF_GROUPS) {
        ln.group = p.group;
        if (p.tune) BA_TRY(tune_group_size(ctx, k, p, ln, &ln.group));
        return launch_gfstack_shared(ctx, k, p, ln, ln.group);
    }
    const int mode = standin ? p.mode_standin : p.mode;

    GfArgs a;
    memset(&a, 0, sizeof(a));
    for (int v = 0; v < k.nvar; v++) {
        a.G[v] = k.libs[v]->g;
        a.slips[v] = k.slips[v];
    }
    a.T = L.T; a.P = L.P; a.N = L.N;
    a.Ttab = Ttab; a.rows_per_target = L.P * L.D * L.S;
    a.tslot = ln.tslot;
    a.C = k.C;
    a.R = R;
    a.order = GfKnobs::get(kn.gf_order, 1);
    a.cgroup = std::max(1, GfKnobs::get(kn.gf_cgroup, 128));
    a.rowoff = ta.rowoff; a.fac = ta.fac;
    a.data = k.data; a.wscalar = k.wscalar; a.out = k.out;
    a.guard = standin;
    const int W = (L.N % 2 == 0) ? 2 : 1;
    const int VEC = 1;
    const int64_t tile_w = (int64_t)256 * W * VEC;
    a.ntile = (int)((L.N + tile_w - 1) / tile_w);
    if (mode == GF_RESID_SCALAR) BA_TRY(ctx->scratch(standin ? SL_PARTIAL2 : SL_PARTIAL, (size_t)k.C * L.T * a.ntile, &a.partial));
    const int64_t nblocks = k.C * L.T * a.ntile;
    BA_CHECK(nblocks < (int64_t)0x7fffffff, BEATAMD_EINVAL, "gfstack: batch too large (%lld blocks)",
             (long long)nblocks);
    a.nblocks = nblocks;
    dim3 grid((unsigned)(standin ? std::min<int64_t>(nblocks, (int64_t)ctx->num_cu * 8) : nblocks));
    if (!standin) {
        snprintf(ctx->last_gf_kernel, sizeof(ctx->last_gf_kernel), "k_gfstack<%d,%d,%d,%d,%d>",
                 k.interp == BEATAMD_MULTILINEAR ? 1 : 0, k.nvar, VEC, W, mode);
        snprintf(ctx->gf_plan, sizeof(ctx->gf_plan), "streaming kernel: %s", k.C < 48 ? "fewer than 48 chains share too few rows" :
                 L.N % 2 ? "odd sample count (the chain-shared kernels move 16-byte lanes)" : "chosen by BEATAMD_GF_KERNEL or no chain-shared kernel fits this library");
        ctx->gs_ngtp = 0;
    }
    {
        ScopedTimer tm(ctx, standin ? "gfstack_standin" : "gfstack");
        const auto launch = k.interp == BEATAMD_NEAREST_NEIGHBOR ? (W == 2 ? launch_nvar<0, 1, 2> : launch_nvar<0, 1, 1>)
                                                                 : (W == 2 ? launch_nvar<1, 1, 2> : launch_nvar<1, 1, 1>);
        launch(k.nvar, mode, grid, ctx->stream, a);
    }
    BA_HIP(hipGetLastError());
    if (mode == GF_RESID_SCALAR) BA_TRY(launch_sum_tiles(ctx, a.partial, k.C * L.T, a.ntile, k.quad, standin, 1));
    if (standin && p.standin_band1)
        BA_TRY(launch_quadform_banded(ctx, k.band_w, 1, L.N, L.T, k.C, k.out, L.T * L.N, L.N, k.quad, L.T, standin, 1));
    return BEATAMD_OK;
}

int launch_gf_tables(beatamd_ctx *ctx, const GfStackCall &k, uint32_t *rowoff, double *fac)
{
    const SeisLib &L = *k.libs[0];
    if (k.C == 0) return BEATAMD_OK;
    BA_CHECK(L.T * L.P * L.D * L.S < (int64_t)0xffffffffLL, BEATAMD_EINVAL, "gfstack: library has more than 2^32 rows");
    BA_CHECK(rowoff && (k.interp != BEATAMD_MULTILINEAR || fac), BEATAMD_EINVAL, "gf_tables: bad argument");
    const int64_t CTP = k.C * L.T * L.P;
    BA_CHECK((CTP + 255) / 256 < (int64_t)0x7fffffff, BEATAMD_EINVAL, "gf_tables: batch too large");
    TabArgs ta;
    ta.interp = k.interp; ta.R = 1;
    ta.C = k.C; ta.T = L.T; ta.P = L.P; ta.D = L.D; ta.S = L.S;
    ta.st_min = L.st_min; ta.st_dt = L.st_dt; ta.du_min = L.du_min; ta.du_dt = L.du_dt;
    ta.durations = k.durations; ta.st = k.st;
    ta.status = ctx->d_status;
    ta.rowoff = rowoff; ta.fac = fac;
    ScopedTimer tm(ctx, "tables");
    hipLaunchKernelGGL(k_gf_tables, dim3((unsigned)((CTP + 255) / 256)), dim3(256), 0, ctx->stream, ta);
    BA_HIP(hipGetLastError());
    return BEATAMD_OK;
}

}
```

beat_amd/csrc/kernels.hpp:

```cpp
#pragma once
#include <algorithm>

#include "ctx.hpp"

namespace beatamd {

constexpr int SWEEP_MAX_CELLS = 6400;
struct SweepLdsPlan {
    int nmax;
    int waves;
    size_t bytes;
};
SweepLdsPlan sweep_lds_plan(int nmax_cells);
int launch_sweep_explicit(beatamd_ctx *ctx, const double *slow, double h, const int32_t *hi,
                          const int32_t *hj, int ni, int nj, int64_t C, double *out);
int launch_sweep_model(beatamd_ctx *ctx, const FfiModel &m, const double *Q, int64_t C,
                       double *starttimes0, int32_t *chain_bad);

struct StartTimeSrc {
    const double *explicit_st = nullptr;
    const double *starttimes0 = nullptr;
    const double *Q = nullptr;
    int64_t nparams = 0;
    const int64_t *shift_off = nullptr;
    int32_t nslot = 0;
    const int32_t *tslot = nullptr;
    const int64_t *slot_shift_off = nullptr;
    int32_t *chain_bad = nullptr;
};

struct ChainVec {
    const double *base = nullptr;
    int64_t stride = 0, off = 0;
};

#ifdef __HIPCC__
__device__ __forceinline__ int64_t xcd_items8(int64_t b, int64_t n)
{
    if (b >= (n & ~(int64_t)63)) return b;
    const int64_t r = b & 63;
    return (b & ~(int64_t)63) + (r & 7) * 8 + (r >> 3);
}
#endif

int gf_patch_ranges(int64_t T, int64_t P, int64_t N, int num_cu);

enum GfMode : int {
    GF_STORE_SYN = 0,
    GF_RESID_SCALAR = 1,
    GF_RESID_STORE = 2,
    GF_RESID_BAND1 = 3
};

struct GfStackCall {
    const SeisLib *libs[4] = {nullptr, nullptr, nullptr, nullptr};
    int nvar = 1;
    ChainVec slips[4];
    ChainVec durations;
    StartTimeSrc st;
    int interp = 0;
    int64_t C = 0;
    int mode = GF_STORE_SYN;
    const double *data = nullptr;
    const double *wscalar = nullptr;
    double *out = nullptr;
    double *quad = nullptr;
    const double *band_w = nullptr;
    bool f32 = false;
    ChainVec order_key[2];
    const int32_t *active = nullptr;
};
int launch_gfstack(beatamd_ctx *ctx, const GfStackCall &call);
int launch_sum_tiles(beatamd_ctx *ctx, const double *partial, int64_t n, int ntile, double *quad, const int *guard = nullptr,
                     int want = 0, const double *edges = nullptr, const double *band_w = nullptr, int64_t T = 1, int64_t N = 0);
int launch_round_to_f32(beatamd_ctx *ctx, double *g, float *g32, int64_t n);
enum GfBand1 : int { GF_BY_NONE, GF_BY_COMBINE, GF_BY_RUNS, GF_BY_WS, GF_BY_QUADFORM };
inline GfBand1 gf_band1(bool carries, GfBand1 by, int *mode)
{
    if (!carries) *mode = GF_RESID_STORE;
    return carries ? by : GF_BY_QUADFORM;
}
enum GfStacker : int { GF_STREAMING, GF_RUNS, GF_GROUPS };
struct GfGroup {
    int cg = 0, ucap = 0, mode = 0;
    bool ws = false;
    GfBand1 band1 = GF_BY_NONE;
};
struct GfPlan {
    const GfKnobs *knobs = nullptr;
    int R = 1;
    int64_t T = 0, P = 0;
    bool tinv = false, slots = false;
    int64_t Ttab = 0;
    int nrow = 1;
    bool f32 = false, pair64 = false, fused = true, ws512 = false;
    GfStacker stacker = GF_STREAMING;
    int mode = 0, mode_standin = 0, mode_combine = 0;
    bool standin_band1 = false;
    GfBand1 band1 = GF_BY_NONE;
    GfGroup group, cand[4];
    int ncand = 0;
    bool tune = false;
};
GfPlan gf_plan_call(const GfStackCall &call, const GfKnobs &kn, int num_cu);
struct GfLaunch {
    const int32_t *tslot = nullptr;
    const uint32_t *rowoff = nullptr;
    const double *fac = nullptr;
    GfGroup group;
};
void gs_record_stats(beatamd_ctx *ctx, const GfStackCall &k, int64_t GTP, int64_t Ttab, int cg, bool has_passes);
bool gfstack_shared_plan(const GfStackCall &call, GfPlan &p);
GfGroup gfstack_group(const GfPlan &p, int cg, int ucap);
int launch_gfstack_shared(beatamd_ctx *ctx, const GfStackCall &call, const GfPlan &p, const GfLaunch &ln, const GfGroup &g);

int launch_chain_members(beatamd_ctx *ctx, int64_t C, const ChainVec key[2], int64_t cg, int64_t ngroups, const uint32_t **members,
                         int strips = 0);
bool gfstack_ml_applicable(const GfStackCall &call, const GfPlan &p);
int launch_gfstack_ml(beatamd_ctx *ctx, const GfStackCall &call, const GfPlan &p, const GfLaunch &ln, const int **ovf);

struct QuadformCall {
    const double *A = nullptr;
    int64_t a_stride = 0;
    int64_t M = 0, nd = 0, C = 0;
    const double *X = nullptr;
    int64_t xs_c = 0, xs_d = 0;
    int upper_tri = 0;
    double *quad = nullptr;
    int64_t q_stride = 0;
};
int launch_quadform(beatamd_ctx *ctx, const QuadformCall &call);
constexpr int QF_BAND_LIMIT = 16;
int launch_band_detect(beatamd_ctx *ctx, const double *A, int64_t nd, int64_t M, void *scratch, int64_t *band_host,
                       double *dropped_rel_host);
int launch_band_pack(beatamd_ctx *ctx, const double *A, int64_t nd, int64_t M, int64_t band, double *wb);
int launch_quadform_banded(beatamd_ctx *ctx, const double *wb, int64_t band, int64_t M, int64_t nd, int64_t C, const double *X,
                           int64_t xs_c, int64_t xs_d, double *quad, int64_t q_stride, const int *guard = nullptr, int want = 0);
struct QuadformSmallCall {
    int nd = 0;
    const double *A[8];
    int64_t M[8], xoff[8];
    int upper_tri[8];
    const double *slog[8];
    const int64_t *hp_off[8];
    int64_t C = 0;
    const double *X = nullptr;
    int64_t xs_c = 0;
    const double *Q = nullptr;
    int64_t nparams = 0;
    double *LL = nullptr;
    int64_t ld = 0;
    bool misfit_only = false;
};
bool quadform_small_applicable(int nd, const int64_t *M);
int launch_quadform_small(beatamd_ctx *ctx, const QuadformSmallCall &call);
int launch_check_upper_tri(beatamd_ctx *ctx, const double *A, int64_t nd, int64_t M, int *flag_dev);

struct HpSrc {
    const double *base = nullptr;
    int64_t stride = 0;
    const int64_t *offs = nullptr;
};
int launch_mvn_finish(beatamd_ctx *ctx, int64_t C, int64_t nd, int64_t M, const double *quad,
                      const double *slog, HpSrc hp, double *logpts, int64_t ld);
int launch_scalar_quad(beatamd_ctx *ctx, int64_t C, int64_t nd, int64_t M, const double *X,
                       int64_t xs_c, int64_t xs_d, const double *w, double *quad);
int launch_geo_stack(beatamd_ctx *ctx, const GeoLib *const *libs, int nvar, int64_t C, const ChainVec *slips, int accumulate,
                     double *mu);
int launch_geo_residual(beatamd_ctx *ctx, int64_t C, int64_t Nobs, const double *data,
                        const double *odw, const double *mu, double *res, const double *Q = nullptr,
                        int64_t nparams = 0, GeoCorr gc = GeoCorr());

int launch_pole_coef(beatamd_ctx *ctx, const PoleTerm *terms, int npole, const double *Q, int64_t nparams, int64_t C, double *out);
int launch_pole_coupling(beatamd_ctx *ctx, const PoleTerm &term, const double *Q, int64_t nparams, int64_t C, int64_t P,
                         const double *Bp, int64_t uparr_off, double *euler_slips, double *coupling);

constexpr int POL_OUT_LLK = 0, POL_OUT_AMP = 1, POL_OUT_M6 = 2;
struct PolArgs {
    PolSource src;
    int32_t nmap = 0, mode = POL_OUT_LLK, ntab = 0, pad_ = 0;
    int64_t NT = 0;
    int64_t map_end[POL_MAX_MAPS] = {};
    int64_t hp_off[POL_MAX_MAPS] = {};
    double hp_fix[POL_MAX_MAPS] = {};
    double gamma = 0.2;
    const double *rw = nullptr, *obs = nullptr, *utab = nullptr, *btab = nullptr;
    const double *Q = nullptr;
    int64_t nparams = 0, C = 0;
    const int32_t *active = nullptr;
    double *out = nullptr;
    int64_t ld = 0;
};
int launch_polarity(beatamd_ctx *ctx, const PolArgs &a);
int launch_w_to_beta(beatamd_ctx *ctx, int64_t n, const double *w, const double *utab, const double *btab, int ntab, double *out);

#ifdef __HIPCC__
template <bool UNIFORM>
__device__ __forceinline__ double geo_corr_subtract(const GeoCorr &gc, const double *Qc, const double *Pc, int64_t k, double r)
// ... 315 lines not shown
```

beat_amd/csrc/model.cpp:

```cpp
#include "model.hpp"

namespace beatamd {

int wset_quad(beatamd_ctx *ctx, const WeightSet &w, int64_t C, const double *X, int64_t xs_c, int64_t xs_d, double *quad)
{
    if (w.kind == BEATAMD_W_SCALAR)
        return launch_scalar_quad(ctx, C, w.nd, w.M, X, xs_c, xs_d, w.w.get(), quad);
    if (wset_banded(ctx, w))
        return launch_quadform_banded(ctx, w.wb.get(), w.band, w.M, w.nd, C, X, xs_c, xs_d, quad, w.nd);
    QuadformCall q;
    q.A = w.w.get(); q.a_stride = w.M * w.M; q.M = w.M; q.nd = w.nd; q.C = C;
    q.X = X; q.xs_c = xs_c; q.xs_d = xs_d; q.upper_tri = w.upper_tri;
    q.quad = quad; q.q_stride = w.nd;
    return launch_quadform(ctx, q);
}

int64_t model_ndata(const FfiModel &m)
{
    int64_t n = 0;
    for (auto &w : m.wavemaps) n += w.T;
    if (m.has_geo) n += (int64_t)m.geo.sizes.size();
    return n;
}

int64_t model_nterm(const FfiModel &m) { return model_ndata(m) + (m.lap >= 0 ? m.layout.nvar : 0); }

void drop_obs_quads(beatamd_ctx *ctx)
{
    for (auto &m : ctx->models)
        if (m) m->obs_quads_valid = false;
}

int model_check_layout(const FfiModel &m)
{
    const beatamd_ffi_layout &L = m.layout;
    const int64_t np = L.nparams;
    BA_CHECK(np > 0, BEATAMD_EINVAL, "layout: nparams must be positive");
    for (int v = 0; v < L.nvar; v++)
        BA_CHECK(L.slip_off[v] >= 0 && L.slip_off[v] + m.P <= np, BEATAMD_EINVAL, "layout: slip variable %d outside q", v);
    if (!m.wavemaps.empty()) {
        BA_CHECK(L.durations_off >= 0 && L.durations_off + m.P <= np, BEATAMD_EINVAL, "layout: durations outside q");
        BA_CHECK(L.velocities_off >= 0 && L.velocities_off + m.P <= np, BEATAMD_EINVAL, "layout: velocities outside q");
        BA_CHECK(L.nuc_strike_off >= 0 && L.nuc_strike_off + m.nsub <= np && L.nuc_dip_off >= 0 &&
                     L.nuc_dip_off + m.nsub <= np && L.time_off >= 0 && L.time_off + m.nsub <= np,
                 BEATAMD_EINVAL, "layout: hypocentre variables outside q");
    }
    BA_CHECK(!m.wavemaps.empty() || m.has_geo || m.has_pol || m.lap >= 0, BEATAMD_EINVAL, "model has no composite");
    return BEATAMD_OK;
}

int stack_all(beatamd_ctx *ctx, const SeisLib &lib, int64_t C, const double *durations, const double *starttimes,
              const double *slips, int interp, double *out)
{
    GfStackCall k;
    k.libs[0] = &lib; k.nvar = 1; k.interp = interp; k.C = C;
    k.slips[0] = ChainVec{slips, lib.P, 0}; k.durations = ChainVec{durations, lib.P, 0};
    k.st.explicit_st = starttimes; k.mode = GF_STORE_SYN; k.out = out;
    return launch_gfstack(ctx, k);
}

int model_start_times(beatamd_ctx *ctx, const FfiModel &m, int64_t C, const double *Q, double **st0, int32_t **chain_bad)
{
    BA_TRY(ctx->scratch(SL_CHAINBAD, (size_t)C, chain_bad));
    BA_HIP(hipMemsetAsync(*chain_bad, 0, (size_t)C * sizeof(int32_t), ctx->stream));
    BA_TRY(ctx->scratch(SL_ST0, (size_t)C * m.P, st0));
    return launch_sweep_model(ctx, m, Q, C, *st0, *chain_bad);
}

int wavemap_call(beatamd_ctx *ctx, const FfiModel &m, const Wavemap &wm, int64_t C, const double *Q, const double *st0,
                 int32_t *chain_bad, GfStackCall *call)
{
    GfStackCall &k = *call;
    const int64_t np = m.layout.nparams;
    k.nvar = m.layout.nvar;
    for (int v = 0; v < k.nvar; v++) {
        k.libs[v] = get_obj(ctx->seislibs, wm.libs[v]);
        BA_CHECK(k.libs[v] && k.libs[v]->g, BEATAMD_EINVAL, "wavemap refers to a destroyed / empty GF library");
        k.slips[v] = ChainVec{Q, np, m.layout.slip_off[v]};
    }
    k.durations = ChainVec{Q, np, m.layout.durations_off};
    k.st.starttimes0 = st0;
    k.st.Q = Q;
    k.st.nparams = np;
    k.order_key[0] = ChainVec{Q, np, m.layout.nuc_strike_off};
    k.order_key[1] = ChainVec{Q, np, m.layout.nuc_dip_off};
    k.st.shift_off = wm.shift_off.get();
    k.st.nslot = wm.nslot; k.st.tslot = wm.tslot.get(); k.st.slot_shift_off = wm.slot_shift_off.get();
    k.st.chain_bad = chain_bad;
    k.interp = wm.interp;
    k.f32 = wm.f32;
    k.C = C;
    k.data = wm.data.get();
    return BEATAMD_OK;
}

int geo_pole_coefficients(beatamd_ctx *ctx, const Geodetic &g, int64_t C, const double *Q, int64_t np, GeoCorr *gc)
{
    *gc = g.corr;
    if (g.corr.npole == 0 || C == 0) return BEATAMD_OK;
    if (C > g.pole_chains) {
        hipStreamCaptureStatus cap = hipStreamCaptureStatusNone;
        BA_HIP(hipStreamIsCapturing(ctx->stream, &cap));
        BA_CHECK(cap == hipStreamCaptureStatusNone, BEATAMD_EINVAL,
                 "pole coefficients: %lld chains inside a graph capture, the buffer holds %lld (run one step before the capture)",
                 (long long)C, (long long)g.pole_chains);
        BA_HIP(hipStreamSynchronize(ctx->stream));
        g.pole_chains = 0;
        BA_TRY(g.pole_coef.alloc((size_t)C * g.corr.npole * 4));
        g.pole_chains = C;
    }
    gc->pole = g.pole_coef.get();
    return launch_pole_coef(ctx, g.corr.pole_terms, g.corr.npole, Q, np, C, g.pole_coef.get());
}

int geodetic_residual(beatamd_ctx *ctx, const FfiModel &m, int64_t C, const double *Q, double *mu_out, double *res_out)
{
    const Geodetic &g = m.geo;
    const int64_t np = m.layout.nparams;
    if (!Q) {
        BA_HIP(hipMemsetAsync(mu_out, 0, (size_t)g.Nobs * sizeof(double), ctx->stream));
        return launch_geo_residual(ctx, 1, g.Nobs, g.data.get(), g.odws.get(), mu_out, res_out);
    }
    if (m.geo_is_geometry) {
        if (!res_out) return launch_geom_los(ctx, m.geom, Q, np, C, mu_out);
        GeoCorr gc;
        BA_TRY(geo_pole_coefficients(ctx, g, C, Q, np, &gc));
        return launch_geom_los(ctx, m.geom, Q, np, C, nullptr, g.data.get(), g.odws.get(), res_out, gc);
    }
    const GeoLib *gls[4] = {nullptr, nullptr, nullptr, nullptr};
    ChainVec slips[4];
    BA_CHECK(m.layout.nvar <= 4, BEATAMD_EINVAL, "geodetic composite: more than 4 slip variables");
    for (int v = 0; v < m.layout.nvar; v++) {
        gls[v] = get_obj(ctx->geolibs, g.libs[v]);
        BA_CHECK(gls[v], BEATAMD_EINVAL, "geodetic composite refers to a destroyed GF library");
        slips[v] = ChainVec{Q, np, m.layout.slip_off[v]};
    }
    BA_TRY(launch_geo_stack(ctx, gls, m.layout.nvar, C, slips, 0, mu_out));
    if (!res_out) return BEATAMD_OK;
    GeoCorr gc;
    BA_TRY(geo_pole_coefficients(ctx, g, C, Q, np, &gc));
    return launch_geo_residual(ctx, C, g.Nobs, g.data.get(), g.odws.get(), mu_out, res_out, Q, np, gc);
}

int laplacian_quad(beatamd_ctx *ctx, const Laplacian &lap, int64_t C, int64_t nvar, const double *slips, double *quad)
{
    QuadformCall q;
    q.A = lap.L.get(); q.a_stride = 0; q.M = lap.P; q.nd = nvar; q.C = C;
    q.X = slips; q.xs_c = nvar * lap.P; q.xs_d = lap.P;
    q.quad = quad; q.q_stride = nvar;
    return launch_quadform(ctx, q);
}

static int geodetic_wset(beatamd_ctx *ctx, const Geodetic &g, size_t d, WeightSet **ws)
{
    *ws = get_obj(ctx->wsets, g.wsets[d]);
    BA_CHECK(*ws && (*ws)->nd == 1 && (*ws)->M == g.sizes[d], BEATAMD_EINVAL,
             "geodetic dataset %zu: weight set missing or of the wrong size", d);
    return BEATAMD_OK;
}

void polarity_call(const Polarity &p, int64_t C, const double *Q, int64_t np, PolArgs *a)
{
    a->src = p.src; a->nmap = p.nmap; a->ntab = p.ntab; a->NT = p.NT;
    for (int i = 0; i < POL_MAX_MAPS; i++) {
        a->map_end[i] = p.map_end[i]; a->hp_off[i] = p.hp_off[i]; a->hp_fix[i] = p.hp_fix[i];
    }
    a->gamma = p.gamma;
    a->rw = p.rw.get(); a->obs = p.obs.get(); a->utab = p.utab.get(); a->btab = p.btab.get();
// ... 356 lines not shown
```

include/beat_amd.h:

```cpp
#ifndef BEAT_AMD_H
#define BEAT_AMD_H

#include <stdint.h>

#ifdef __cplusplus
extern "C" {
#endif

#define BEATAMD_OK 0
#define BEATAMD_EINVAL (-1)
#define BEATAMD_EHIP (-2)
#define BEATAMD_EINDEX (-3)
#define BEATAMD_ENOMEM (-4)
#define BEATAMD_ENAN (-5)
#define BEATAMD_ENOTPSD (-6)
#define BEATAMD_EOUTSIDE (-8)
#define BEATAMD_EBADCOV (-7)

#define BEATAMD_VERSION 120

#define BEATAMD_NEAREST_NEIGHBOR 0
#define BEATAMD_MULTILINEAR 1

#define BEATAMD_W_SCALAR 0
#define BEATAMD_W_DENSE 1

#define BEATAMD_DOMAIN_TIME 0
#define BEATAMD_DOMAIN_SPECTRUM 1

typedef struct beatamd_ctx beatamd_ctx;

const char *beatamd_last_error(void);
int beatamd_version(void);

int beatamd_ctx_create(int device, beatamd_ctx **out);
int beatamd_ctx_destroy(beatamd_ctx *ctx);
int beatamd_ctx_set_stream(beatamd_ctx *ctx, void *hip_stream);
int beatamd_ctx_use_own_stream(beatamd_ctx *ctx);
int beatamd_ctx_synchronize(beatamd_ctx *ctx);
int beatamd_ctx_reload_knobs(beatamd_ctx *ctx);
int beatamd_ctx_set_step_counter(beatamd_ctx *ctx, uint32_t *device_counter);
int beatamd_ctx_enable_timing(beatamd_ctx *ctx, int on);
int beatamd_ctx_kernel_time(beatamd_ctx *ctx, const char *kernel, double *total_ms,
                            int64_t *launches);
int beatamd_ctx_reset_timing(beatamd_ctx *ctx);
int beatamd_ctx_last_kernel(beatamd_ctx *ctx, char *buf, int64_t buflen);
int beatamd_ctx_gf_group_stats(beatamd_ctx *ctx, int64_t *chains_per_group, double *mean_rows,
                               int64_t *max_rows, int64_t *row_bytes);
int beatamd_ctx_gf_plan(beatamd_ctx *ctx, char *buf, int64_t buflen, double *mean_passes, int64_t *max_passes);
int beatamd_ctx_gf_tune_log(beatamd_ctx *ctx, char *buf, int64_t buflen);
int32_t beatamd_gf_patch_ranges(int64_t ntargets, int64_t npatches, int64_t nsamples, int32_t num_cu);
int beatamd_ffi_start_times_batch(beatamd_ctx *ctx, int32_t model_id, int64_t C, const double *Q, double *times,
                                  int32_t *chain_bad);
int beatamd_ffi_magnitudes_batch(beatamd_ctx *ctx, int32_t model_id, int64_t C, const double *Q, const double *moment_per_slip,
                                 const int64_t *comp_off, int32_t ncomp, double *M0, double *Mw);
int beatamd_ffi_moment_rate_spans_batch(beatamd_ctx *ctx, int32_t model_id, int64_t C, const double *Q,
                                        const double *start_times, const int32_t *chain_bad, double deltat, int64_t *spans);
#define BEATAMD_STF_HALF_SINUSOID 0
int beatamd_ffi_moment_rates_batch(beatamd_ctx *ctx, int32_t model_id, int64_t C, const double *Q, const double *moment_per_slip,
                                   const int64_t *comp_off, int32_t ncomp, const double *start_times, const int32_t *chain_bad,
                                   double deltat, int32_t stf, int64_t kbase, int64_t NT, double *rates, int64_t *spans);
int32_t beatamd_fast_sweep_lds(int32_t ncells, int32_t *waves);
int beatamd_seis_gflib_set_split_targets(beatamd_ctx *ctx, int32_t lib_id, int64_t ntargets);

int beatamd_ctx_gf_chain_groups(beatamd_ctx *ctx, int64_t C, const double *key0, const double *key1,
                                int64_t chains_per_group, uint32_t *members);

int beatamd_fast_sweep_batch(beatamd_ctx *ctx, const double *slowness, double patch_size,
                             const int32_t *h_strk, const int32_t *h_dip, int32_t num_strk,
                             int32_t num_dip, int64_t C, double *out);

int beatamd_seis_gflib_create(beatamd_ctx *ctx, int64_t ntargets, int64_t npatches,
                              int64_t ndurations, int64_t nstarttimes, int64_t nsamples,
                              double starttime_min, double starttime_sampling,
                              double duration_min, double duration_sampling, int32_t *lib_id);
int beatamd_seis_gflib_upload(beatamd_ctx *ctx, int32_t lib_id, const double *src,
                              int64_t offset, int64_t count);
int beatamd_seis_gflib_adopt(beatamd_ctx *ctx, int32_t lib_id, double *device_ptr);
int beatamd_seis_gflib_round_to_f32(beatamd_ctx *ctx, int32_t lib_id);
int beatamd_ffi_model_set_f32(beatamd_ctx *ctx, int32_t model_id, int32_t wavemap_index, int32_t on);
int beatamd_seis_gflib_device_ptr(beatamd_ctx *ctx, int32_t lib_id, double **device_ptr);
int beatamd_seis_gflib_destroy(beatamd_ctx *ctx, int32_t lib_id);

int beatamd_seis_stack_all_batch(beatamd_ctx *ctx, int32_t lib_id, int64_t C,
                                 const double *durations, const double *starttimes,
                                 const double *slips, int32_t interpolation, double *out);

int beatamd_geo_gflib_create(beatamd_ctx *ctx, int64_t npatches, int64_t nobs, const double *G,
                             int32_t *lib_id);
int beatamd_geo_gflib_destroy(beatamd_ctx *ctx, int32_t lib_id);
int beatamd_geo_stack_all_batch(beatamd_ctx *ctx, int32_t lib_id, int64_t C,
                                const double *slips, int32_t accumulate, double *out);

int beatamd_geo_ensemble_create(beatamd_ctx *ctx, const int32_t *lib_ids, int64_t K, int64_t nvar, int32_t *ens_id);
int beatamd_geo_ensemble_destroy(beatamd_ctx *ctx, int32_t ens_id);
int beatamd_geo_ensemble_stack(beatamd_ctx *ctx, int32_t ens_id, const double *slips, double *X);
int beatamd_pred_covariance_batch(beatamd_ctx *ctx, int64_t K, int64_t Nobs, const double *X, int64_t nd,
                                  const int64_t *sizes, const double *const *base, double *const *out);

int beatamd_weights_create(beatamd_ctx *ctx, int32_t kind, int64_t ndatasets, int64_t M,
                           const double *weights, const double *slog_pdet, int32_t *wset_id);
int beatamd_weights_update(beatamd_ctx *ctx, int32_t wset_id, int32_t kind, int64_t count,
                           const double *weights, const double *slog_pdet);
int beatamd_weights_destroy(beatamd_ctx *ctx, int32_t wset_id);
int beatamd_weights_band(beatamd_ctx *ctx, int32_t wset_id, int64_t *band);
int beatamd_weights_band_info(beatamd_ctx *ctx, int32_t wset_id, int64_t *band, double *max_dropped_rel);
int beatamd_mvn_chol_logp_batch(beatamd_ctx *ctx, int32_t wset_id, int64_t C,
                                const double *residuals, const double *hp, double *logpts);

int beatamd_laplacian_create(beatamd_ctx *ctx, int64_t npatches, const double *L,
                             double logdet, int32_t *lap_id);
int beatamd_laplacian_destroy(beatamd_ctx *ctx, int32_t lap_id);
int beatamd_laplacian_logp_batch(beatamd_ctx *ctx, int32_t lap_id, int64_t C, int64_t nvar,
                                 const double *slips, const double *hp, double *out);

typedef struct beatamd_ffi_layout {
    int64_t nparams;
    int32_t nvar;
    int64_t slip_off[4];
    int64_t durations_off;
    int64_t velocities_off;
    int64_t nuc_strike_off;
    int64_t nuc_dip_off;
    int64_t time_off;
    int64_t h_laplacian_off;
} beatamd_ffi_layout;

int beatamd_ffi_model_create(beatamd_ctx *ctx, const beatamd_ffi_layout *layout,
                             int32_t nsubfaults, const int32_t *n_patch_dip,
                             const int32_t *n_patch_strike, const double *patch_size,
                             int32_t *model_id);
int beatamd_ffi_model_add_wavemap(beatamd_ctx *ctx, int32_t model_id, const int32_t *lib_ids,
                                  const double *data, int32_t wset_id, const int64_t *hp_off,
                                  const int64_t *shift_off, int32_t interpolation);
int beatamd_ffi_model_add_wavemap_spectrum(beatamd_ctx *ctx, int32_t model_id, const int32_t *lib_ids,
                                           const double *data_spec, int32_t wset_id, const int64_t *hp_off,
                                           const int64_t *shift_off, int32_t interpolation, int64_t ntrans, int64_t lo,
                                           int64_t hi);
int beatamd_amp_spectrum_batch(beatamd_ctx *ctx, int64_t R, int64_t N, int64_t ntrans, int64_t lo, int64_t hi,
                               const double *X, const double *data_spec, int64_t T, double *out);
int beatamd_ffi_model_add_geodetic(beatamd_ctx *ctx, int32_t model_id, const int32_t *geo_lib_ids,
                                   const double *data, const double *odws, int32_t ndatasets,
                                   const int64_t *dataset_sizes, const int32_t *wset_ids,
                                   const int64_t *hp_off);
int beatamd_ffi_model_add_geodetic_geometry(beatamd_ctx *ctx, int32_t model_id, int32_t nsrc,
                                            const int32_t *kind, const int64_t *param_off,
                                            const double *param_fixed, int64_t nobs,
                                            const double *east, const double *north,
                                            const double *los, double nu, const double *data,
// ... 237 lines not shown
```

Measured before the change: 93080 chain-steps/s.

## Add paired-row f64 consumer to chain-shared gfstack kernel with windowed chain ordering

```diff
diff --git a/beat_amd/_lib.py b/beat_amd/_lib.py
--- a/beat_amd/_lib.py
+++ b/beat_amd/_lib.py
@@ -112,6 +112,9 @@
     "beatamd_seis_gflib_set_split_targets": [_vp, _i32, _i64],
     "beatamd_ctx_reload_knobs": [_vp],
     "beatamd_ctx_gf_chain_groups": [_vp, _i64, _vp, _vp, _i64, _vp],
+    "beatamd_ctx_ws_windows": [_vp, _pi32],
+    "beatamd_ctx_ws_order": [_vp, _i64, _vp, _vp, _f64, _i32, _i32, _vp, _vp],
+    "beatamd_ctx_ws_slot_tables": [_vp, _i64, _i64, _i64, _i64, _vp, _vp, _i32, _pi64, _pi32, _vp, _vp, _vp, _vp],
     "beatamd_smc_calc_beta": [_vp, _i64, _vp, _i64, _f64, _f64, C.POINTER(_f64), _vp],
     "beatamd_smc_stage_weights": [_vp, _i64, _vp, _i64, _f64, _vp],
     "beatamd_smc_resample": [_vp, _i64, _vp, _f64, _vp],
diff --git a/beat_amd/csrc/capi.cpp b/beat_amd/csrc/capi.cpp
--- a/beat_amd/csrc/capi.cpp
+++ b/beat_amd/csrc/capi.cpp
@@ -2153,6 +2153,42 @@
     BA_HIP(hipStreamSynchronize(ctx->stream));
     BA_HIP(hipMemcpy(members, m, (size_t)(ngroups * chains_per_group) * sizeof(uint32_t), hipMemcpyDeviceToHost));
     return BEATAMD_OK;
+}
+
+int beatamd_ctx_ws_windows(beatamd_ctx *ctx, int32_t *windows)
+{
+    ENTER(ctx);
+    BA_CHECK(windows != nullptr, BEATAMD_EINVAL, "ws_windows: bad argument");
+    *windows = ctx->gs_windows;
+    return BEATAMD_OK;
+}
+
+int beatamd_ctx_ws_order(beatamd_ctx *ctx, int64_t C, const double *key_strike, const double *key_dip, double patch_size,
+                         int32_t ndip, int32_t nstrike, const int32_t *active, uint32_t *members)
+{
+    ENTER(ctx);
+    BA_CHECK(C > 0 && members && (key_strike != nullptr) == (key_dip != nullptr), BEATAMD_EINVAL, "ws_order: bad argument");
+    Staging st(ctx);
+    const double *d_ks, *d_kd;
+    const int32_t *d_act;
+    BA_TRY(st.in(key_strike, (size_t)C, &d_ks));
+    BA_TRY(st.in(key_dip, (size_t)C, &d_kd));
+    BA_TRY(st.in(active, (size_t)C, &d_act));
+    return ws_order_alone(ctx, C, d_ks, d_kd, patch_size, ndip, nstrike, d_act, members);
+}
+
+int beatamd_ctx_ws_slot_tables(beatamd_ctx *ctx, int64_t C, int64_t T, int64_t P, int64_t DS, const uint32_t *rowoff,
+                               const uint32_t *order, int32_t pair, int64_t *vmax, int32_t *cap, uint32_t *nv, uint16_t *slot,
+                               uint32_t *uent, uint32_t *ucount)
+{
+    ENTER(ctx);
+    BA_CHECK(C > 0 && T > 0 && P > 0 && DS > 0 && rowoff && vmax && cap && (!slot || (nv && uent && ucount)), BEATAMD_EINVAL,
+             "ws_slot_tables: bad argument");
+    Staging st(ctx);
+    const uint32_t *d_row, *d_ord;
+    BA_TRY(st.in(rowoff, (size_t)(C * T * P), &d_row));
+    BA_TRY(st.in(order, (size_t)(((C + 511) / 512) * 512), &d_ord));
+    return ws_tables_alone(ctx, C, T, P, DS, d_row, d_ord, pair, vmax, cap, nv, slot, uent, ucount);
 }
 
 int beatamd_smc_calc_beta(beatamd_ctx *ctx, int64_t C, const double *likelihoods, int64_t stride,
diff --git a/beat_amd/csrc/ctx.hpp b/beat_amd/csrc/ctx.hpp
--- a/beat_amd/csrc/ctx.hpp
+++ b/beat_amd/csrc/ctx.hpp
@@ -315,6 +315,7 @@
     int64_t gs_ngtp = 0, gs_N = 0;
     double gs_trep = 1;
     int gs_nvar = 1;
+    int gs_windows = 0;
     bool gs_has_passes = false;
     char gf_plan[384] = "";
     char gf_tune_log[512] = "";
diff --git a/beat_amd/csrc/gfshared.hip b/beat_amd/csrc/gfshared.hip
--- a/beat_amd/csrc/gfshared.hip
+++ b/beat_amd/csrc/gfshared.hip
@@ -782,13 +782,130 @@
     asm("s_waitcnt lgkmcnt(12)\n\t" BA_FMA4A BA_RD4A(OFFNEXT) "s_waitcnt lgkmcnt(12)\n\t" BA_FMA4B BA_RD4B(OFFNEXT) \
         : BA_ACC8(G), BA_Y8(Y) : "v"(w), "v"(xs))
 
-template <int NROW, int MODE, int NB, int NTH>
+#define F2_FMA(G, Y)                                                          \
+    _Pragma("unroll") for (int q = 0; q < 4; q++) {                           \
+        acc[(G) * 8 + 2 * q] = fma((double)Y[q].x, w, acc[(G) * 8 + 2 * q]);   \
+        acc[(G) * 8 + 2 * q + 1] = fma((double)Y[q].y, w, acc[(G) * 8 + 2 * q + 1]); \
+    }
+#define F2_GROUP(F32_, G, Y, OFFNEXT)              \
+    lds_wait4_pair<4>(Y);                      \
+    __builtin_amdgcn_sched_barrier(0);       \
+    F2_FMA(G, Y)                             \
+    __builtin_amdgcn_sched_barrier(0);       \
+    lds_rd4_pair<F32_ ? 1 : 2, OFFNEXT>(Y, xs, s);           \
+    __builtin_amdgcn_sched_barrier(0);
+#define GS_PAIR_CONSUMER(F32_)                                                                                                     \
+                                         \
+    uint32_t sl_n;                                                                                                                 \
+    double wl_n;                                                                                                                   \
+    const uint32_t voff_s = (uint32_t)tid * 2u;                                                                                    \
+    const char *const slot_base = reinterpret_cast<const char *>(a.slot + (gt * a.vmax) * CG);                                     \
+    const char *const w_base = reinterpret_cast<const char *>(a.w + (gt * a.vmax) * CG);                                           \
+    const uint32_t slot_step = (uint32_t)(CG * 2);                                                                                 \
+    const uint32_t w_step = (uint32_t)(CG * 8);                                                                                    \
+    const int64_t w_var_bytes = a.w_var_stride * 8;                                                                                \
+    auto tab_slot = [&](int p) { return slot_base + (uint32_t)p * slot_step; };                                                    \
+    auto tab_w = [&](int p, int iv) {                                                                                              \
+        return w_base + (uint32_t)p * w_step + (nvar == 1 ? (int64_t)0 : (int64_t)iv * w_var_bytes);                               \
+    };                                                                                                                             \
+    auto fetch_tabs = [&](const char *ps, const char *pw) {                                                                        \
+        asm("global_load_ushort %0, %1, %2" : "=v"(sl_n) : "v"(voff_s), "s"(ps));                                                  \
+        uint32_t voff_w;                                                                                                           \
+        asm("v_lshlrev_b32 %1, 2, %2\n\t"                                                                                          \
+            "global_load_dwordx2 %0, %1, %3" : "=v"(wl_n), "=&v"(voff_w) : "v"(voff_s), "s"(pw));                                  \
+    };                                                                                                                             \
+                                        \
+    auto row_address = [&](uint32_t base) {                                                                                        \
+        uint32_t x;                                                                                                                \
+        asm("s_waitcnt vmcnt(0)\n\t"                                                                                               \
+            "v_lshl_add_u32 %0, %1, 5, %1\n\t"                                                                                     \
+            "v_lshl_add_u32 %0, %0, %c4, %2" : "=&v"(x) : "v"(sl_n), "s"(base), "v"(wl_n), "n"(F32_ ? 3 : 4));                     \
+        return x;                                                                                                                  \
+    };                                                                                                                             \
+    auto landed_weight = [&](uint32_t after) {                                 \
+        double x;                                                                                                                  \
+        asm("v_mov_b64 %0, %1" : "=v"(x) : "v"(wl_n), "v"(after));                                                                 \
+        return x;                                                                                                                  \
+    };                                                                                                                             \
+    static_assert(GS_PITCH == 66, "row_address multiplies by 33 qwords");                                                          \
+    static_assert(GS_NT == 64, "the read schedule below is written for 64-sample tiles");                                          \
+                            \
+                            \
+                     \
+                                  \
+                                                                                  \
+    typedef typename std::conditional<F32_ != 0, v2f, v2d>::type gs_pair_t;                                                        \
+    gs_pair_t ya[4], yb[4];                                                                                                        \
+    int p1 = 0, iv1 = 0;                                              \
+    gs_advance(p1, iv1, P, nvar);                                                                                                  \
+    int gbuf = 0;                                                                       \
+    const int ring = NB * bufsz;                                                                                                   \
+    double w;                                                                                                                      \
+    uint32_t xs;                                                                                                                   \
+                                   \
+    if (F32_ == 0 && __ballot(c < a.C) == 0) {                                                                                     \
+        for (int s = 0; s <= nsteps; s++) __builtin_amdgcn_s_barrier();                                                            \
+    } else {                                                                                                                       \
+    fetch_tabs(tab_slot(0), tab_w(0, 0));                                                                                          \
+    xs = row_address(lds0);                                                                                                        \
+    w = landed_weight(xs);                                                                                                         \
+    __builtin_amdgcn_sched_barrier(0);                                                                                             \
+    __builtin_amdgcn_s_barrier();                                                                      \
+    __builtin_amdgcn_sched_barrier(0);                                                                                             \
+    lds_rd4_pair<F32_ ? 1 : 2, 0>(ya, xs, -1);                                                                                     \
+    lds_rd4_pair<F32_ ? 1 : 2, 32>(yb, xs, -1);                                                                                    \
+    __builtin_amdgcn_sched_barrier(0);                                                                                             \
+    fetch_tabs(tab_slot(p1), tab_w(p1, iv1));                                                                                      \
+    gs_advance(p1, iv1, P, nvar);                                                                                                  \
+    _Pragma("clang loop unroll(disable)")                                                                                          \
+    for (int s = 0; s < nsteps; s++) {                                                                                             \
+        int gnext = gbuf + bufsz;                                                                                                  \
+        if (gnext == ring) gnext = 0;                                                                                              \
+        const char *const ps2 = tab_slot(p1), *const pw2 = tab_w(p1, iv1);                                 \
+        gs_advance(p1, iv1, P, nvar);                                                                                              \
+        __builtin_amdgcn_sched_barrier(0);                                                                                         \
+        F2_GROUP(F32_, 0, ya, 64)                                                                                                  \
+        F2_GROUP(F32_, 1, yb, 96)                                                                                                  \
+        F2_GROUP(F32_, 2, ya, 128)                                                                                                 \
+        F2_GROUP(F32_, 3, yb, 160)                                                                                                 \
+        F2_GROUP(F32_, 4, ya, 192)                                                                                                 \
+        F2_GROUP(F32_, 5, yb, 224)                                                                                                 \
+                                              \
+        lds_wait4_pair<0>(ya);                                                                                                     \
+        lds_wait4_pair<0>(yb);                                                                                                     \
+        __builtin_amdgcn_sched_barrier(0);                                                                                         \
+        F2_FMA(6, ya)                                                                                                              \
+        __builtin_amdgcn_sched_barrier(0);                                                                                         \
+        gbuf = gnext;                                                                                                              \
+        const uint32_t xs_n = row_address(lds0 + (uint32_t)(gbuf * (F32_ ? 4 : 8)));    \
+        __builtin_amdgcn_sched_barrier(0);                                                                                         \
+        __builtin_amdgcn_s_barrier();                          \
+        __builtin_amdgcn_sched_barrier(0);                                                                                         \
+        lds_rd4_pair<F32_ ? 1 : 2, 0>(ya, xs_n, s);                \
+        __builtin_amdgcn_sched_barrier(0);                                                                                         \
+                                  \
+        F2_FMA(7, yb)                                                                                                              \
+        __builtin_amdgcn_sched_barrier(0);                                                                                         \
+        w = landed_weight(xs_n);                                                                                                   \
+        lds_rd4_pair<F32_ ? 1 : 2, 32>(yb, xs_n, s);                                                                               \
+        xs = xs_n;                                                                                                                 \
+        __builtin_amdgcn_sched_barrier(0);                                                                                         \
+        fetch_tabs(ps2, pw2);                                                                       \
+    }                                                                                                                              \
+                                \
+    asm volatile("s_waitcnt vmcnt(0) lgkmcnt(0)"                                                                                   \
+                 : "+v"(ya[0]), "+v"(ya[1]), "+v"(ya[2]), "+v"(ya[3]), "+v"(yb[0]), "+v"(yb[1]), "+v"(yb[2]),                      \
+                   "+v"(yb[3]), "+v"(sl_n), "+v"(wl_n));                                                                           \
+    __builtin_amdgcn_sched_barrier(0);                                                                                             \
+    }
+
+template <int NROW, int MODE, int NB, int NTH, int PAIR>
 __global__ void __launch_bounds__(768) __attribute__((amdgpu_waves_per_eu(3, 3)))
 k_gfstack_ws(GsArgs a)
 {
     constexpr int CW = 8, LW = 4;
     constexpr int GS_NT = 64;
-    constexpr int GS_PITCH = GS_NT + 1;
+    constexpr int GS_PITCH = GS_NT + (PAIR ? 2 : 1);
     constexpr int KPRE = 16;
     extern __shared__ __attribute__((aligned(16))) double xbuf[];
     constexpr int CG = CW * 64;
@@ -817,6 +934,9 @@
     double acc[GS_NT];
 #pragma unroll
     for (int i = 0; i < GS_NT; i++) acc[i] = 0.0;
+    if constexpr (PAIR != 0) {
+    GS_PAIR_CONSUMER(0)
+    } else {
     uint32_t sl_n;
     double wl_n;
     const uint32_t voff_s = (uint32_t)tid * 2u;
@@ -923,6 +1043,7 @@
                    "+v"(yb[6]), "+v"(yb[7]), "+v"(sl_n), "+v"(wl_n));
     __builtin_amdgcn_sched_barrier(0);
     }
+    }
 
     const bool live = (c < a.C);
     const int nvalid = (int)min((int64_t)GS_NT, N - n0);
@@ -1026,107 +1147,7 @@
     double acc[GS_NT];
 #pragma unroll
     for (int i = 0; i < GS_NT; i++) acc[i] = 0.0;
-    uint32_t sl_n;
-    double wl_n;
-    const uint32_t voff_s = (uint32_t)tid * 2u;
-    const char *const slot_base = reinterpret_cast<const char *>(a.slot + (gt * a.vmax) * CG);
-    const char *const w_base = reinterpret_cast<const char *>(a.w + (gt * a.vmax) * CG);
-    const uint32_t slot_step = (uint32_t)(CG * 2);
-    const uint32_t w_step = (uint32_t)(CG * 8);
-    const int64_t w_var_bytes = a.w_var_stride * 8;
-    auto tab_slot = [&](int p) { return slot_base + (uint32_t)p * slot_step; };
-    auto tab_w = [&](int p, int iv) {
-        return w_base + (uint32_t)p * w_step + (nvar == 1 ? (int64_t)0 : (int64_t)iv * w_var_bytes);
-    };
-    auto fetch_tabs = [&](const char *ps, const char *pw) {
-        asm("global_load_ushort %0, %1, %2" : "=v"(sl_n) : "v"(voff_s), "s"(ps));
-        uint32_t voff_w;
-        asm("v_lshlrev_b32 %1, 2, %2\n\t"
-            "global_load_dwordx2 %0, %1, %3" : "=v"(wl_n), "=&v"(voff_w) : "v"(voff_s), "s"(pw));
-    };
-    auto row_address = [&](uint32_t base) {
-        uint32_t x;
-        asm("s_waitcnt vmcnt(0)\n\t"
-            "v_lshl_add_u32 %0, %1, 5, %1\n\t"
-            "v_lshl_add_u32 %0, %0, %c4, %2" : "=&v"(x) : "v"(sl_n), "s"(base), "v"(wl_n), "n"(F32 ? 3 : 4));
-        return x;
-    };
-    auto landed_weight = [&](uint32_t after) {
-        double x;
-        asm("v_mov_b64 %0, %1" : "=v"(x) : "v"(wl_n), "v"(after));
-        return x;
-    };
-    static_assert(GS_PITCH == 66, "row_address multiplies by 33 qwords");
-    static_assert(GS_NT == 64, "the read schedule below is written for 64-sample tiles");
-    pair_t ya[4], yb[4];
-    int p1 = 0, iv1 = 0;
-    gs_advance(p1, iv1, P, nvar);
-    int gbuf = 0;
-    const int ring = NB * bufsz;
-    double w;
-    uint32_t xs;
-    fetch_tabs(tab_slot(0), tab_w(0, 0));
-    xs = row_address(lds0);
-    w = landed_weight(xs);
-    __builtin_amdgcn_sched_barrier(0);
-    __builtin_amdgcn_s_barrier();
-    __builtin_amdgcn_sched_barrier(0);
-    lds_rd4_pair<F32 ? 1 : 2, 0>(ya, xs, -1);
-    lds_rd4_pair<F32 ? 1 : 2, 32>(yb, xs, -1);
-    __builtin_amdgcn_sched_barrier(0);
-    fetch_tabs(tab_slot(p1), tab_w(p1, iv1));
-    gs_advance(p1, iv1, P, nvar);
-#define F2_FMA(G, Y)                                                          \
-    _Pragma("unroll") for (int q = 0; q < 4; q++) {                           \
-        acc[(G) * 8 + 2 * q] = fma((double)Y[q].x, w, acc[(G) * 8 + 2 * q]);   \
-        acc[(G) * 8 + 2 * q + 1] = fma((double)Y[q].y, w, acc[(G) * 8 + 2 * q + 1]); \
-    }
-#define F2_GROUP(G, Y, OFFNEXT)              \
-    lds_wait4_pair<4>(Y);                      \
-    __builtin_amdgcn_sched_barrier(0);       \
-    F2_FMA(G, Y)                             \
-    __builtin_amdgcn_sched_barrier(0);       \
-    lds_rd4_pair<F32 ? 1 : 2, OFFNEXT>(Y, xs, s);           \
-    __builtin_amdgcn_sched_barrier(0);
-#pragma clang loop unroll(disable)
-    for (int s = 0; s < nsteps; s++) {
-        int gnext = gbuf + bufsz;
-        if (gnext == ring) gnext = 0;
-        const char *const ps2 = tab_slot(p1), *const pw2 = tab_w(p1, iv1);
-        gs_advance(p1, iv1, P, nvar);
-        __builtin_amdgcn_sched_barrier(0);
-        F2_GROUP(0, ya, 64)
-        F2_GROUP(1, yb, 96)
-        F2_GROUP(2, ya, 128)
-        F2_GROUP(3, yb, 160)
-        F2_GROUP(4, ya, 192)
-        F2_GROUP(5, yb, 224)
-        lds_wait4_pair<0>(ya);
-        lds_wait4_pair<0>(yb);
-        __builtin_amdgcn_sched_barrier(0);
-        F2_FMA(6, ya)
-        __builtin_amdgcn_sched_barrier(0);
-        gbuf = gnext;
-        const uint32_t xs_n = row_address(lds0 + (uint32_t)(gbuf * ES));
-        __builtin_amdgcn_sched_barrier(0);
-        __builtin_amdgcn_s_barrier();
-        __builtin_amdgcn_sched_barrier(0);
-        lds_rd4_pair<F32 ? 1 : 2, 0>(ya, xs_n, s);
-        __builtin_amdgcn_sched_barrier(0);
-        F2_FMA(7, yb)
-        __builtin_amdgcn_sched_barrier(0);
-        w = landed_weight(xs_n);
-        lds_rd4_pair<F32 ? 1 : 2, 32>(yb, xs_n, s);
-        xs = xs_n;
-        __builtin_amdgcn_sched_barrier(0);
-        fetch_tabs(ps2, pw2);
-    }
-#undef F2_GROUP
-#undef F2_FMA
-    asm volatile("s_waitcnt vmcnt(0) lgkmcnt(0)"
-                 : "+v"(ya[0]), "+v"(ya[1]), "+v"(ya[2]), "+v"(ya[3]), "+v"(yb[0]), "+v"(yb[1]), "+v"(yb[2]),
-                   "+v"(yb[3]), "+v"(sl_n), "+v"(wl_n));
-    __builtin_amdgcn_sched_barrier(0);
+    GS_PAIR_CONSUMER(F32)
 
     const bool live = (c < a.C);
     const int nvalid = (int)min((int64_t)GS_NT, N - n0);
@@ -1149,6 +1170,10 @@
     }
 }
 
+#undef GS_PAIR_CONSUMER
+#undef F2_GROUP
+#undef F2_FMA
+
 
 template <int WAVES, int NROW, int MODE>
 static int launch_shared_one(dim3 grid, size_t lds, hipStream_t s, const GsArgs &a)
@@ -1194,10 +1219,16 @@
 #define BA_WS_PICK0(NAME, ...)                                                                         \
     (mode == GF_STORE_SYN ? NAME<__VA_ARGS__ GF_STORE_SYN, 3, 0>                                      \
      : mode == GF_RESID_SCALAR ? NAME<__VA_ARGS__ GF_RESID_SCALAR, 3, 0> : NAME<__VA_ARGS__ GF_RESID_STORE, 3, 0>)
+#define BA_WS_PICKP(NTH_, PAIR_)                                                                        \
+    (mode == GF_STORE_SYN ? k_gfstack_ws<1, GF_STORE_SYN, 3, NTH_, PAIR_>                             \
+     : mode == GF_RESID_SCALAR ? k_gfstack_ws<1, GF_RESID_SCALAR, 3, NTH_, PAIR_> : k_gfstack_ws<1, GF_RESID_STORE, 3, NTH_, PAIR_>)
     if (pair == 1) kern = a.nthint ? BA_WS_PICK(k_gfstack_wsp, 1,) : BA_WS_PICK0(k_gfstack_wsp, 1,);
     else if (pair == 2) kern = a.nthint ? BA_WS_PICK(k_gfstack_wsp, 0,) : BA_WS_PICK0(k_gfstack_wsp, 0,);
-    else if (mode == GF_RESID_BAND1) kern = a.nthint ? k_gfstack_ws<1, GF_RESID_BAND1, 3, 1> : k_gfstack_ws<1, GF_RESID_BAND1, 3, 0>;
-    else kern = a.nthint ? BA_WS_PICK(k_gfstack_ws, 1,) : BA_WS_PICK0(k_gfstack_ws, 1,);
+    else if (pair == 3)
+        kern = a.nthint ? k_gfstack_ws<1, GF_RESID_SCALAR, 3, 1, 1> : k_gfstack_ws<1, GF_RESID_SCALAR, 3, 0, 1>;
+    else if (mode == GF_RESID_BAND1) kern = a.nthint ? k_gfstack_ws<1, GF_RESID_BAND1, 3, 1, 0> : k_gfstack_ws<1, GF_RESID_BAND1, 3, 0, 0>;
+    else kern = a.nthint ? BA_WS_PICKP(1, 0) : BA_WS_PICKP(0, 0);
+#undef BA_WS_PICKP
 #undef BA_WS_PICK0
 #undef BA_WS_PICK
     BA_HIP(hipFuncSetAttribute((const void *)kern, hipFuncAttributeMaxDynamicSharedMemorySize, (int)lds));
@@ -1213,6 +1244,7 @@
 
 struct WsTabArgs {
     int nvar, cap;
+    int win;
     int64_t C, T, P, DS;
     int64_t vmax;
     const uint32_t *rowoff;
@@ -1253,29 +1285,48 @@
     if (tid == 0) nv[gt] = run;
 }
 
-__global__ void __launch_bounds__(WS_CG) k_ws_pack(const uint32_t *order, const int32_t *active, int64_t C, uint32_t *out)
-{
-    __shared__ uint32_t wsum[WS_CG / 64];
+constexpr int WS_KEY_BAND = 4;
+struct WsPackKey {
+    ChainVec strike, dip;
+    double h;
+    int ndip, nstrike;
+};
+
+__global__ void __launch_bounds__(WS_CG) k_ws_pack(const uint32_t *order, const int32_t *active, int64_t C, WsPackKey kk, uint32_t *out)
+{
+    __shared__ __attribute__((aligned(16))) uint32_t keys[WS_CG];
     const int tid = threadIdx.x;
-    const int lane = tid & 63, wv = tid >> 6;
     const int64_t pos = (int64_t)blockIdx.x * WS_CG + tid;
     const uint32_t c = order ? order[pos] : (pos < C ? (uint32_t)pos : 0xffffffffu);
-    const bool on = c != 0xffffffffu && (int64_t)c < C && active[c] != 0;
-    const uint64_t m = __ballot(on);
-    if (lane == 0) wsum[wv] = (uint32_t)__popcll(m);
+    const bool on = c != 0xffffffffu && (int64_t)c < C && (!active || active[c] != 0);
+    uint32_t key = 0;
+    if (on && kk.strike.base) {
+        const double pd = kk.dip.base[(int64_t)c * kk.dip.stride + kk.dip.off];
+        const double ps = kk.strike.base[(int64_t)c * kk.strike.stride + kk.strike.off];
+        const double fi = fmin(fmax(rint((pd - kk.h / 2.0) / kk.h), 0.0), (double)(kk.ndip - 1));
+        const double fj = fmin(fmax(rint((ps - kk.h / 2.0) / kk.h), 0.0), (double)(kk.nstrike - 1));
+        const int band = (int)fi / WS_KEY_BAND, hj = (int)fj;
+        key = (uint32_t)(band * kk.nstrike + ((band & 1) ? kk.nstrike - 1 - hj : hj));
+    }
+    const uint32_t mine = on ? ((key << 9) | (uint32_t)tid) : (0xfffffe00u | (uint32_t)tid);
+    keys[tid] = mine;
     __syncthreads();
-    uint32_t before = 0, total = 0;
-    for (int q = 0; q < WS_CG / 64; q++) {
-        const uint32_t x = wsum[q];
-        if (q < wv) before += x;
-        total += x;
-    }
-    uint32_t *o = out + (int64_t)blockIdx.x * WS_CG;
-    if (on) o[before + (uint32_t)__popcll(m & ((1ull << lane) - 1ull))] = c;
-    if ((uint32_t)tid >= total) o[tid] = 0xffffffffu;
+    uint32_t rank = 0;
+    const uint4 *k4 = reinterpret_cast<const uint4 *>(keys);
+    for (int q = 0; q < WS_CG / 4; q++) {
+        const uint4 x = k4[q];
+        rank += (x.x < mine) + (x.y < mine) + (x.z < mine) + (x.w < mine);
+    }
+    out[(int64_t)blockIdx.x * WS_CG + rank] = on ? c : 0xffffffffu;
 }
 
 constexpr int64_t WS_MAP_MAX = 16384;
+__device__ inline int ws_pair_lane_group(int tid)
+{
+    const int l = tid & 31;
+    const int set = ((l >= 4 && l < 12) || (l >= 16 && l < 20) || l >= 28) ? 1 : 0;
+    return (tid >> 6) * 4 + ((tid >> 5) & 1) * 2 + set;
+}
 template <int FILL, int MAP>
 __global__ void __launch_bounds__(WS_CG) k_ws_tables(WsTabArgs a)
 {
@@ -1376,16 +1427,17 @@
     if constexpr (!MAP) {
         if (first) lst[pos] = v;
     }
-    if (live) atomicOr(&gm[pos], 1u << (tid >> 5));
+    if (live) atomicOr(&gm[pos], 1u << (a.win == 32 ? (tid >> 5) : ws_pair_lane_group(tid)));
     __syncthreads();
     const int mypass = live ? (int)pos / per : -1;
     if (wv < npass) {
         const int base = wv * per;
         const int n = min(per, (int)U - base);
-        if (n <= 32) {
+        const int W = a.win;
+        if (n <= W) {
             if (lane < n) slt[base + lane] = (uint16_t)lane;
         } else {
-            const int depth = a.cap / 32;
+            const int depth = a.cap / W;
             const int r0 = lane, r1 = lane + 64;
             const uint32_t m0 = r0 < n ? gm[base + r0] : 0u, m1 = r1 < n ? gm[base + r1] : 0u;
             const int key0 = r0 < n ? ((__popc(m0) << 8) | (255 - r0)) : -1;
@@ -1396,25 +1448,25 @@
                 rank0 += kj > key0;
                 rank1 += kj > key1;
             }
-            if (r0 < n && rank0 < 32) slt[base + r0] = (uint16_t)rank0;
-            if (r1 < n && rank1 < 32) slt[base + r1] = (uint16_t)rank1;
+            if (r0 < n && rank0 < W) slt[base + r0] = (uint16_t)rank0;
+            if (r1 < n && rank1 < W) slt[base + r1] = (uint16_t)rank1;
             if (r0 < n) rk2i[wv][rank0] = (uint8_t)r0;
             if (r1 < n) rk2i[wv][rank1] = (uint8_t)r1;
             wave_lds_sync();
             uint32_t wmask = 0;
             int wcnt = 0;
-            if (lane < 32) {
+            if (lane < W) {
                 wmask = gm[base + rk2i[wv][lane]];
                 wcnt = 1;
             }
-            for (int rk = 32; rk < n; rk++) {
+            for (int rk = W; rk < n; rk++) {
                 const int ridx = (int)rk2i[wv][rk];
                 const uint32_t mm = gm[base + ridx];
-                int cost = (lane < 32 && wcnt < depth) ? ((__popc(wmask & mm) << 12) | (wcnt << 6) | lane) : 0x7fffffff;
+                int cost = (lane < W && wcnt < depth) ? ((__popc(wmask & mm) << 12) | (wcnt << 6) | lane) : 0x7fffffff;
                 cost = wave_butterfly<OpMin>(cost);
                 const int w = cost & 63;
                 if (lane == w) {
-                    slt[base + ridx] = (uint16_t)(w + 32 * wcnt);
+                    slt[base + ridx] = (uint16_t)(w + W * wcnt);
                     wmask |= mm;
                     wcnt++;
                 }
@@ -1545,6 +1597,109 @@
     ctx->gs_cg = cg;
     ctx->gs_nvar = k.nvar;
     ctx->gs_has_passes = has_passes;
+    ctx->gs_windows = 0;
+}
+
+int launch_ws_order(beatamd_ctx *ctx, const GfStackCall &k, const GfKnobs &kn, bool by_hypocentre, const uint32_t **order)
+{
+    const int64_t ngroups = (k.C + WS_CG - 1) / WS_CG;
+    const bool keys = k.order_key[0].base && k.order_key[1].base;
+    *order = nullptr;
+    if (ngroups > 1 && keys && GfKnobs::get(kn.gc_global, 1) != 0)
+        BA_TRY(launch_chain_members(ctx, k.C, k.order_key, WS_CG, ngroups, order, GfKnobs::get(kn.gc_global, 1) == 2));
+    WsPackKey kk;
+    memset(&kk, 0, sizeof(kk));
+    if (by_hypocentre && keys && k.key_h > 0.0 && k.key_ndip > 0 && k.key_nstrike > 0 &&
+        (int64_t)((k.key_ndip + WS_KEY_BAND - 1) / WS_KEY_BAND) * k.key_nstrike < ((int64_t)1 << 22)) {
+        kk.strike = k.order_key[0]; kk.dip = k.order_key[1];
+        kk.h = k.key_h; kk.ndip = k.key_ndip; kk.nstrike = k.key_nstrike;
+    }
+    if (k.active || kk.strike.base) {
+        uint32_t *packed;
+        BA_TRY(ctx->scratch(SL_WS_PACK, (size_t)ngroups * WS_CG, &packed));
+        hipLaunchKernelGGL(k_ws_pack, dim3((unsigned)ngroups), dim3(WS_CG), 0, ctx->stream, *order, k.active, k.C, kk, packed);
+        *order = packed;
+    }
+    return BEATAMD_OK;
+}
+
+int launch_ws_tables(beatamd_ctx *ctx, WsTabArgs &ta, int64_t GT, int maxpass, const GfKnobs &kn, uint32_t **nv_out)
+{
+    const int64_t GTP = GT * ta.P;
+    BA_TRY(ctx->scratch(SL_GS_UCOUNT, (size_t)(3 * GTP + GT), &ta.utotal));
+    ta.npass = ta.utotal + GTP;
+    uint32_t *voff = ta.npass + GTP, *nv = voff + GTP;
+    const size_t nvs = (size_t)GT * ta.vmax + 3;
+    BA_TRY(ctx->scratch(SL_GS_UROWS, nvs, &ta.ucount));
+    BA_TRY(ctx->scratch(SL_GS_USLOT, nvs * WS_USTRIDE * 2, &ta.uent));
+    BA_TRY(ctx->scratch(SL_GS_SLOT, nvs * WS_CG, &ta.slot));
+    ta.w_var_stride = (int64_t)GT * ta.vmax * WS_CG;
+    BA_TRY(ctx->scratch(SL_GS_W, (size_t)ta.w_var_stride * ta.nvar + (size_t)3 * WS_CG, &ta.w));
+    const bool map = ta.DS <= WS_MAP_MAX && !GfKnobs::is(kn.ws_map, 0);
+    const size_t mlds = map ? (size_t)ta.DS * sizeof(uint16_t) : 0;
+    if (maxpass > 1) {
+        if (map) hipLaunchKernelGGL((k_ws_tables<0, 1>), dim3((unsigned)GTP), dim3(WS_CG), mlds, ctx->stream, ta);
+        else hipLaunchKernelGGL((k_ws_tables<0, 0>), dim3((unsigned)GTP), dim3(WS_CG), 0, ctx->stream, ta);
+        hipLaunchKernelGGL(k_ws_scan, dim3((unsigned)GT), dim3(256), 0, ctx->stream, ta.npass, voff, nv, ta.P);
+        ta.voff = voff;
+    }
+    if (map) hipLaunchKernelGGL((k_ws_tables<1, 1>), dim3((unsigned)GTP), dim3(WS_CG), mlds, ctx->stream, ta);
+    else hipLaunchKernelGGL((k_ws_tables<1, 0>), dim3((unsigned)GTP), dim3(WS_CG), 0, ctx->stream, ta);
+    *nv_out = nv;
+    return BEATAMD_OK;
+}
+
+static void ws_cap(int64_t DS, int *cap, int *maxpass)
+{
+    const int64_t bound = std::min<int64_t>(WS_CG, DS);
+    *cap = bound <= 32 ? 32 : bound <= 64 ? 64 : WS_CAP_MAX;
+    *maxpass = (int)((bound + *cap - 1) / *cap);
+}
+
+int ws_order_alone(beatamd_ctx *ctx, int64_t C, const double *key_strike, const double *key_dip, double h, int ndip, int nstrike,
+                   const int32_t *active, uint32_t *members)
+{
+    GfStackCall k;
+    k.C = C; k.active = active;
+    if (key_strike && key_dip) {
+        k.order_key[0] = ChainVec{key_strike, 1, 0};
+        k.order_key[1] = ChainVec{key_dip, 1, 0};
+        k.key_h = h; k.key_ndip = ndip; k.key_nstrike = nstrike;
+    }
+    const uint32_t *order = nullptr;
+    BA_TRY(launch_ws_order(ctx, k, gf_knobs(ctx), true, &order));
+    BA_HIP(hipGetLastError());
+    BA_HIP(hipStreamSynchronize(ctx->stream));
+    const int64_t n = ((C + WS_CG - 1) / WS_CG) * WS_CG;
+    if (order) BA_HIP(hipMemcpy(members, order, (size_t)n * sizeof(uint32_t), hipMemcpyDeviceToHost));
+    else for (int64_t i = 0; i < n; i++) members[i] = i < C ? (uint32_t)i : 0xffffffffu;
+    return BEATAMD_OK;
+}
+
+int ws_tables_alone(beatamd_ctx *ctx, int64_t C, int64_t T, int64_t P, int64_t DS, const uint32_t *rowoff, const uint32_t *order,
+                    int pair, int64_t *vmax_out, int32_t *cap_out, uint32_t *nv, uint16_t *slot, uint32_t *uent, uint32_t *ucount)
+{
+    WsTabArgs ta;
+    memset(&ta, 0, sizeof(ta));
+    int maxpass = 1;
+    ws_cap(DS, &ta.cap, &maxpass);
+    ta.win = pair ? 16 : 32;
+    ta.C = C; ta.T = T; ta.P = P; ta.DS = DS; ta.vmax = P * maxpass;
+    ta.rowoff = rowoff; ta.order = order; ta.R = 1;
+    *vmax_out = ta.vmax; *cap_out = ta.cap;
+    if (!slot) return BEATAMD_OK;
+    const int64_t GT = ((C + WS_CG - 1) / WS_CG) * T;
+    uint32_t *nvp = nullptr;
+    BA_TRY(launch_ws_tables(ctx, ta, GT, maxpass, gf_knobs(ctx), &nvp));
+    BA_HIP(hipGetLastError());
+    BA_HIP(hipStreamSynchronize(ctx->stream));
+    const size_t nvs = (size_t)(GT * ta.vmax);
+    if (maxpass > 1) BA_HIP(hipMemcpy(nv, nvp, (size_t)GT * sizeof(uint32_t), hipMemcpyDeviceToHost));
+    else for (int64_t i = 0; i < GT; i++) nv[i] = (uint32_t)P;
+    BA_HIP(hipMemcpy(slot, ta.slot, nvs * WS_CG * sizeof(uint16_t), hipMemcpyDeviceToHost));
+    BA_HIP(hipMemcpy(uent, ta.uent, nvs * WS_USTRIDE * 2 * sizeof(uint32_t), hipMemcpyDeviceToHost));
+    BA_HIP(hipMemcpy(ucount, ta.ucount, nvs * sizeof(uint32_t), hipMemcpyDeviceToHost));
+    return BEATAMD_OK;
 }
 
 static int launch_gfstack_ws(beatamd_ctx *ctx, const GfStackCall &k, const GfPlan &p, const GfLaunch &ln, const GfGroup &g)
@@ -1555,47 +1710,24 @@
     const int mode = g.mode;
     const int64_t ngroups = (k.C + WS_CG - 1) / WS_CG;
     const int64_t GT = ngroups * Ttab, GTP = GT * L.P;
-    const int64_t bound = std::min<int64_t>(WS_CG, L.D * L.S);
-    const int cap = bound <= 32 ? 32 : bound <= 64 ? 64 : WS_CAP_MAX;
-    const int maxpass = (int)((bound + cap - 1) / cap);
+    int cap, maxpass;
+    ws_cap(L.D * L.S, &cap, &maxpass);
     const int64_t vmax = L.P * maxpass;
 
     WsTabArgs ta;
     memset(&ta, 0, sizeof(ta));
     ta.nvar = k.nvar; ta.cap = cap;
+    const bool ws_pair = !p.f32 && (p.pair64 || (p.ws_pair && mode == GF_RESID_SCALAR && ngroups == 1 && maxpass == 1 && p.R == 1));
+    ta.win = ws_pair ? 16 : 32;
     ta.C = k.C; ta.T = Ttab; ta.P = L.P; ta.DS = L.D * L.S; ta.vmax = vmax;
     ta.rowoff = ln.rowoff;
     for (int v = 0; v < k.nvar; v++) ta.slips[v] = k.slips[v];
     ta.R = p.R;
-    if (ngroups > 1 && k.order_key[0].base && k.order_key[1].base && GfKnobs::get(kn.gc_global, 1) != 0)
-        BA_TRY(launch_chain_members(ctx, k.C, k.order_key, WS_CG, ngroups, &ta.order, GfKnobs::get(kn.gc_global, 1) == 2));
-    BA_TRY(ctx->scratch(SL_GS_UCOUNT, (size_t)(3 * GTP + GT), &ta.utotal));
-    ta.npass = ta.utotal + GTP;
-    uint32_t *voff = ta.npass + GTP, *nv = voff + GTP;
-    const size_t nvs = (size_t)GT * vmax + 3;
-    BA_TRY(ctx->scratch(SL_GS_UROWS, nvs, &ta.ucount));
-    BA_TRY(ctx->scratch(SL_GS_USLOT, nvs * WS_USTRIDE * 2, &ta.uent));
-    BA_TRY(ctx->scratch(SL_GS_SLOT, nvs * WS_CG, &ta.slot));
-    ta.w_var_stride = (int64_t)GT * vmax * WS_CG;
-    BA_TRY(ctx->scratch(SL_GS_W, (size_t)ta.w_var_stride * k.nvar + (size_t)3 * WS_CG, &ta.w));
+    uint32_t *nv = nullptr;
     {
         ScopedTimer tm(ctx, "grouptables");
-        if (k.active) {
-            uint32_t *packed;
-            BA_TRY(ctx->scratch(SL_WS_PACK, (size_t)ngroups * WS_CG, &packed));
-            hipLaunchKernelGGL(k_ws_pack, dim3((unsigned)ngroups), dim3(WS_CG), 0, ctx->stream, ta.order, k.active, k.C, packed);
-            ta.order = packed;
-        }
-        const bool map = ta.DS <= WS_MAP_MAX && !GfKnobs::is(kn.ws_map, 0);
-        const size_t mlds = map ? (size_t)ta.DS * sizeof(uint16_t) : 0;
-        if (maxpass > 1) {
-            if (map) hipLaunchKernelGGL((k_ws_tables<0, 1>), dim3((unsigned)GTP), dim3(WS_CG), mlds, ctx->stream, ta);
-            else hipLaunchKernelGGL((k_ws_tables<0, 0>), dim3((unsigned)GTP), dim3(WS_CG), 0, ctx->stream, ta);
-            hipLaunchKernelGGL(k_ws_scan, dim3((unsigned)GT), dim3(256), 0, ctx->stream, ta.npass, voff, nv, L.P);
-            ta.voff = voff;
-        }
-        if (map) hipLaunchKernelGGL((k_ws_tables<1, 1>), dim3((unsigned)GTP), dim3(WS_CG), mlds, ctx->stream, ta);
-        else hipLaunchKernelGGL((k_ws_tables<1, 0>), dim3((unsigned)GTP), dim3(WS_CG), 0, ctx->stream, ta);
+        BA_TRY(launch_ws_order(ctx, k, kn, ws_pair, &ta.order));
+        BA_TRY(launch_ws_tables(ctx, ta, GT, maxpass, kn, &nv));
     }
     BA_HIP(hipGetLastError());
 
@@ -1619,7 +1751,7 @@
     const int64_t nblocks = gs_grid(a, kn);
     BA_CHECK(nblocks < (int64_t)0x7fffffff, BEATAMD_EINVAL, "gfstack: batch too large");
     size_t lds = f32 ? (size_t)(cap + 1) * (64 + 2) * sizeof(float) * 3
-                     : (size_t)(cap + 1) * (64 + (pair64 ? 2 : 1)) * sizeof(double) * 3;
+                     : (size_t)(cap + 1) * (64 + (ws_pair ? 2 : 1)) * sizeof(double) * 3;
     lds = std::max<size_t>(lds, (64 + 8 * 64 * 17) * sizeof(double));
     BA_CHECK(lds <= 160 * 1024, BEATAMD_EINVAL, "internal: k_gfstack_ws row buffers exceed LDS");
     if (f32 || pair64)
@@ -1632,9 +1764,10 @@
              "D*S = %lld) rows), %s", cap, (long long)(L.D * L.S),
              maxpass > 1 ? "patches that touch more are staged in passes of equal size" : "one pass per patch");
     gs_record_stats(ctx, k, GTP, Ttab, WS_CG, maxpass > 1);
+    ctx->gs_windows = f32 ? 0 : ta.win;
     {
         ScopedTimer tm(ctx, "gfstack");
-        BA_TRY(launch_ws(mode, dim3((unsigned)nblocks), lds, ctx->stream, a, f32 ? 1 : (pair64 ? 2 : 0)));
+        BA_TRY(launch_ws(mode, dim3((unsigned)nblocks), lds, ctx->stream, a, f32 ? 1 : pair64 ? 2 : ws_pair ? 3 : 0));
     }
     BA_HIP(hipGetLastError());
     if (a.partial)
diff --git a/beat_amd/csrc/gfstack.hip b/beat_amd/csrc/gfstack.hip
--- a/beat_amd/csrc/gfstack.hip
+++ b/beat_amd/csrc/gfstack.hip
@@ -418,6 +418,7 @@
     p.f32 = k.f32;
     for (int v = 0; v < k.nvar; v++) p.f32 = p.f32 && k.libs[v]->g32 != nullptr;
     p.pair64 = GfKnobs::is(kn.gs_pair, 1);
+    p.ws_pair = !GfKnobs::is(kn.gs_pair, 0);
     p.fused = !GfKnobs::is(kn.qf_fuse, 0);
     p.mode = p.R > 1 ? (int)GF_STORE_SYN : k.mode;
     p.mode_combine = k.mode;
@@ -614,6 +615,7 @@
         snprintf(ctx->gf_plan, sizeof(ctx->gf_plan), "streaming kernel: %s", k.C < 48 ? "fewer than 48 chains share too few rows" :
                  L.N % 2 ? "odd sample count (the chain-shared kernels move 16-byte lanes)" : "chosen by BEATAMD_GF_KERNEL or no chain-shared kernel fits this library");
         ctx->gs_ngtp = 0;
+        ctx->gs_windows = 0;
     }
     {
         ScopedTimer tm(ctx, standin ? "gfstack_standin" : "gfstack");
diff --git a/beat_amd/csrc/kernels.hpp b/beat_amd/csrc/kernels.hpp
--- a/beat_amd/csrc/kernels.hpp
+++ b/beat_amd/csrc/kernels.hpp
@@ -68,6 +68,8 @@
     const double *band_w = nullptr;
     bool f32 = false;
     ChainVec order_key[2];
+    double key_h = 0.0;
+    int key_ndip = 0, key_nstrike = 0;
     const int32_t *active = nullptr;
 };
 int launch_gfstack(beatamd_ctx *ctx, const GfStackCall &call);
@@ -94,6 +96,7 @@
     int64_t Ttab = 0;
     int nrow = 1;
     bool f32 = false, pair64 = false, fused = true, ws512 = false;
+    bool ws_pair = true;
     GfStacker stacker = GF_STREAMING;
     int mode = 0, mode_standin = 0, mode_combine = 0;
     bool standin_band1 = false;
@@ -114,6 +117,10 @@
 GfGroup gfstack_group(const GfPlan &p, int cg, int ucap);
 int launch_gfstack_shared(beatamd_ctx *ctx, const GfStackCall &call, const GfPlan &p, const GfLaunch &ln, const GfGroup &g);
 
+int ws_order_alone(beatamd_ctx *ctx, int64_t C, const double *key_strike, const double *key_dip, double h, int ndip, int nstrike,
+                   const int32_t *active, uint32_t *members);
+int ws_tables_alone(beatamd_ctx *ctx, int64_t C, int64_t T, int64_t P, int64_t DS, const uint32_t *rowoff, const uint32_t *order,
+                    int pair, int64_t *vmax_out, int32_t *cap_out, uint32_t *nv, uint16_t *slot, uint32_t *uent, uint32_t *ucount);
 int launch_chain_members(beatamd_ctx *ctx, int64_t C, const ChainVec key[2], int64_t cg, int64_t ngroups, const uint32_t **members,
                          int strips = 0);
 bool gfstack_ml_applicable(const GfStackCall &call, const GfPlan &p);
diff --git a/beat_amd/csrc/model.cpp b/beat_amd/csrc/model.cpp
--- a/beat_amd/csrc/model.cpp
+++ b/beat_amd/csrc/model.cpp
@@ -84,6 +84,7 @@
     k.st.nparams = np;
     k.order_key[0] = ChainVec{Q, np, m.layout.nuc_strike_off};
     k.order_key[1] = ChainVec{Q, np, m.layout.nuc_dip_off};
+    k.key_h = m.patch_size[0]; k.key_ndip = m.ndip[0]; k.key_nstrike = m.nstrike[0];
     k.st.shift_off = wm.shift_off.get();
     k.st.nslot = wm.nslot; k.st.tslot = wm.tslot.get(); k.st.slot_shift_off = wm.slot_shift_off.get();
     k.st.chain_bad = chain_bad;
diff --git a/beat_amd/wstables.py b/beat_amd/wstables.py
--- /dev/null
+++ b/beat_amd/wstables.py
@@ -0,0 +1,47 @@
+import ctypes as C
+
+import numpy as np
+
+from ._lib import check
+
+NONE = 0xffffffff
+
+
+def _p(a):
+    return None if a is None else a.ctypes.data_as(C.c_void_p)
+
+
+def ws_windows(ctx):
+    w = C.c_int32()
+    check(ctx._lib.beatamd_ctx_ws_windows(ctx._h, C.byref(w)))
+    return w.value
+
+
+def ws_order(ctx, n_chains, key_strike=None, key_dip=None, patch_size=1.0, ndip=0, nstrike=0, active=None):
+    n = int(n_chains)
+    ks = None if key_strike is None else np.ascontiguousarray(key_strike, dtype=np.float64)
+    kd = None if key_dip is None else np.ascontiguousarray(key_dip, dtype=np.float64)
+    act = None if active is None else np.ascontiguousarray(active, dtype=np.int32)
+    ng = (n + 511) // 512
+    out = np.empty(ng * 512, dtype=np.uint32)
+    check(ctx._lib.beatamd_ctx_ws_order(ctx._h, n, _p(ks), _p(kd), float(patch_size), int(ndip), int(nstrike), _p(act), _p(out)))
+    return out.reshape(ng, 512)
+
+
+def ws_slot_tables(ctx, rowoff, n_rows, order=None, pair=False):
+    rowoff = np.ascontiguousarray(rowoff, dtype=np.uint32)
+    Cn, T, P = rowoff.shape
+    ng = (Cn + 511) // 512
+    order = None if order is None else np.ascontiguousarray(order, dtype=np.uint32).reshape(ng * 512)
+    vmax, cap = C.c_int64(), C.c_int32()
+    args = (ctx._h, Cn, T, P, int(n_rows), _p(rowoff), _p(order), 1 if pair else 0, C.byref(vmax), C.byref(cap))
+    check(ctx._lib.beatamd_ctx_ws_slot_tables(*args, None, None, None, None))
+    nvs = ng * T * vmax.value
+    nv = np.empty(ng * T, dtype=np.uint32)
+    slot = np.empty(nvs * 512, dtype=np.uint16)
+    uent = np.empty(nvs * 256, dtype=np.uint32)
+    count = np.empty(nvs, dtype=np.uint32)
+    check(ctx._lib.beatamd_ctx_ws_slot_tables(*args, _p(nv), _p(slot), _p(uent), _p(count)))
+    ent = uent.reshape(ng, T, vmax.value, 4, 32, 2).transpose(0, 1, 2, 4, 3, 5).reshape(ng, T, vmax.value, 128, 2)
+    return dict(cap=cap.value, vmax=vmax.value, nv=nv.reshape(ng, T), slot=slot.reshape(ng, T, vmax.value, 512),
+                rows=ent[..., 0], slots=ent[..., 1], count=count.reshape(ng, T, vmax.value))
diff --git a/include/beat_amd.h b/include/beat_amd.h
--- a/include/beat_amd.h
+++ b/include/beat_amd.h
@@ -65,6 +65,13 @@
 
 int beatamd_ctx_gf_chain_groups(beatamd_ctx *ctx, int64_t C, const double *key0, const double *key1,
                                 int64_t chains_per_group, uint32_t *members);
+
+int beatamd_ctx_ws_windows(beatamd_ctx *ctx, int32_t *windows);
+int beatamd_ctx_ws_order(beatamd_ctx *ctx, int64_t C, const double *key_strike, const double *key_dip, double patch_size,
+                         int32_t ndip, int32_t nstrike, const int32_t *active, uint32_t *members);
+int beatamd_ctx_ws_slot_tables(beatamd_ctx *ctx, int64_t C, int64_t T, int64_t P, int64_t DS, const uint32_t *rowoff,
+                               const uint32_t *order, int32_t pair, int64_t *vmax, int32_t *cap, uint32_t *nv, uint16_t *slot,
+                               uint32_t *uent, uint32_t *ucount);
 
 int beatamd_fast_sweep_batch(beatamd_ctx *ctx, const double *slowness, double patch_size,
                              const int32_t *h_strk, const int32_t *h_dip, int32_t num_strk,
```

Result: faster. 95040 chain-steps/s, median of 6 (+2.1%).
